# safe-autonomous-systems/fluidgym

Hardware: AMD Instinct MI355X
Metric: env-steps/sec (batched) + pressure-Poisson HBM GB/s vs roofline, 1/2/4/8 GPUs (higher is better)
Workload: dtype f32; 1 GPU; ChannelJet2D-v0 (2D channel stand-in for 'cylinder Re=100 256x128'), 64 envs/GPU, 25 PISO steps/env step, random jets, stirred by a body force N(0,2.0) redrawn every env step; global_batch=64, parallelism=env-sharded x1, 1 bcast + 1 all_gather per step (RCCL), lanes_per_gpu=2, workload_modified=True, capped_solves=0, floor_released_solves=0, advection_solver_form=two-brick, velocity_solver=on-chip Jacobi sweeps (policy advection_jacobi; 11972 solves settled by

## Files before the change

fluidgym_amd/_lib.py:

```python
from __future__ import annotations

import ctypes
import os
from ctypes import POINTER, Structure, c_char_p, c_float, c_int, c_int32, c_int64, c_void_p

_HERE = os.path.dirname(os.path.abspath(__file__))
LIB_PATH = os.environ.get("FLUIDGYM_AMD_LIB") or os.path.join(_HERE, "libfluidgym_hip.so")
LIB_F64_PATH = os.environ.get("FLUIDGYM_AMD_LIB_F64") or os.path.join(_HERE, "libfluidgym_hip_f64.so")

FG_MAX_SCALARS = 4
FG_FIELD_SUMMARY_WORK_BYTES = 128
FG_OK = 0
FG_ERR_NOT_CONVERGED = -5
FG_ERR_NOT_FINITE = -6
FG_ERR_FLUX_BALANCE = -7
FG_PERIODIC, FG_FIXED = 0, 1
FG_DIRICHLET, FG_NEUMANN = 0, 1
FG_VELOCITY, FG_PRESSURE, FG_SCALAR, FG_VELOCITY_SOURCE, FG_VISCOSITY_FIELD = 0, 1, 2, 3, 4
FG_BOUND_VELOCITY, FG_BOUND_SCALAR = 8, 16
FG_SOLVER_CG, FG_SOLVER_JACOBI, FG_SOLVER_RBGS, FG_SOLVER_MGCG, FG_SOLVER_FDCG = 0, 1, 2, 3, 4
(FG_BUF_A, FG_BUF_C_OFF, FG_BUF_ADV_RHS, FG_BUF_VEL_RESULT, FG_BUF_H, FG_BUF_DIV, FG_BUF_P_RESULT,
 FG_BUF_SCALAR_RESULT) = range(8)
FG_ERR_UNSUPPORTED = -4
FG_ERR_INVALID_ARG = -1
# ... 210 lines not shown
class FgMbSimOptions(Structure):
    _fields_ = [
        ("step", FgMbStepOptions),
        ("time_step", c_float),
        ("cfl", c_float),
        ("adaptive", c_int32),
        ("substeps", c_int32),
        ("flux_balance_tol", c_float),
        ("outflow_slot0", c_int32),
        ("outflow_count", c_int32),
        ("outflow_velm", c_float * 3),
        ("outflow_tol", c_float),
        ("max_substeps", c_int32),
        ("outflow_slot0_b", c_int32),
        ("outflow_count_b", c_int32),
    ]


(FG_MB_BUF_A, FG_MB_BUF_C_OFF, FG_MB_BUF_RHS, FG_MB_BUF_H, FG_MB_BUF_DIV, FG_MB_BUF_P_DIAG, FG_MB_BUF_P_OFF,
 FG_MB_BUF_VELOCITY_RESULT) = range(8)
FG_MB_BUF_KRYLOV0 = 8
FG_MB_BUF_PRESSURE_X = 13


class FgSimOptions(Structure):
    _fields_ = [
        ("step", FgStepOptions),
        ("time_step", c_float),
        ("cfl", c_float),
        ("adaptive", c_int32),
        ("substeps", c_int32),
        ("flux_balance_tol", c_float),
        ("outflow_mask", c_int32),
        ("outflow_velm", c_float * 3),
        ("outflow_tol", c_float),
        ("max_substeps", c_int32),
    ]


SIGNATURES = {
    "fg_abi_version": (c_int, []),
    "fg_last_error": (c_char_p, []),
    "fg_create": (c_int, [POINTER(FgConfig), POINTER(c_float), POINTER(c_float), POINTER(c_float), POINTER(c_void_p)]),
    "fg_destroy": (c_int, [c_void_p]),
    "fg_bind": (c_int, [c_void_p, c_int, c_void_p]),
    "fg_set_viscosity": (c_int, [c_void_p, c_float]),
    "fg_set_scalar_viscosity": (c_int, [c_void_p, c_int, c_float]),
    "fg_set_viscosity_batch": (c_int, [c_void_p, c_void_p]),
    "fg_set_scalar_viscosity_batch": (c_int, [c_void_p, c_int, c_void_p]),
    "fg_set_fd_preconditioner": (c_int, [c_void_p] + [POINTER(c_float)] * 7),
    "fg_max_velocity": (c_int, [c_void_p, c_void_p, c_void_p]),
    "fg_set_fd_fast_transform": (c_int, [c_void_p, c_int, c_float]),
    "fg_set_return_best": (c_int, [c_void_p, c_int]),
    "fg_set_cg_reset_steps": (c_int, [c_void_p, c_int]),
    "fg_set_advection_start": (c_int, [c_void_p, c_int]),
    "fg_set_wall_stress_forcing": (c_int, [c_void_p, c_int, c_float, c_float]),
    "fg_boundary_flux_balance": (c_int, [c_void_p, c_void_p, c_void_p]),
    "fg_step_diagnostics": (c_int, [c_void_p, POINTER(c_float), c_void_p]),
    "fg_update_advective_boundary": (c_int, [c_void_p, c_int, POINTER(c_float), c_void_p, c_void_p]),
    "fg_balance_boundary_fluxes": (c_int, [c_void_p, c_int, c_float, c_void_p, c_void_p]),
    "fg_setup_advection": (c_int, [c_void_p, c_void_p, c_int, c_int, c_void_p]),
    "fg_solve_advection": (c_int, [c_void_p, c_int, c_int, c_float, c_int, POINTER(FgSolveInfo), c_void_p]),
    "fg_copy_scalar_result_to_blocks": (c_int, [c_void_p, c_int, c_void_p]),
    "fg_setup_pressure_matrix": (c_int, [c_void_p, c_void_p]),
    "fg_setup_pressure_rhs": (c_int, [c_void_p, c_void_p, c_void_p]),
    "fg_solve_pressure": (c_int, [c_void_p, c_int, c_float, c_int, c_int, POINTER(FgSolveInfo), c_void_p]),
    "fg_correct_velocity": (c_int, [c_void_p, c_void_p]),
    "fg_copy_velocity_result_to_blocks": (c_int, [c_void_p, c_void_p]),
    "fg_copy_velocity_result_from_blocks": (c_int, [c_void_p, c_void_p]),
    "fg_piso_step": (c_int, [c_void_p, c_void_p, POINTER(FgStepOptions), POINTER(c_int32), c_void_p]),
    "fg_single_step": (c_int, [c_void_p, POINTER(FgSimOptions), POINTER(c_int32), POINTER(c_float), c_void_p]),
    "fg_multi_step": (c_int, [c_void_p, POINTER(FgSimOptions), c_int32, POINTER(c_void_p), POINTER(c_int32), POINTER(c_float), POINTER(c_int32), c_void_p]),
    "fg_make_divergence_free": (c_int, [c_void_p, c_float, c_int, POINTER(FgSolveInfo), c_void_p]),
    "fg_reset_solver_state": (c_int, [c_void_p, c_void_p]),
    "fg_solver_hints": (c_int, [c_void_p, POINTER(c_int32), c_int32]),
    "fg_env_restore_field": (c_int, [c_void_p, c_int, c_void_p, c_int32, POINTER(FgEnvSel), c_int32, c_int32, c_void_p]),
    "fg_env_reset_solver_state": (c_int, [c_void_p, POINTER(FgEnvSel), c_int32, c_void_p]),
    "fg_mb_env_restore_field": (c_int, [c_void_p, c_int, c_void_p, c_int32, POINTER(FgEnvSel), c_int32, c_int32, c_void_p]),
    "fg_mb_env_reset_solver_state": (c_int, [c_void_p, POINTER(FgEnvSel), c_int32, c_void_p]),
    "fg_mb_restore_envs": (c_int, [c_void_p, c_void_p, c_void_p, c_void_p, c_int32, POINTER(FgEnvSel), c_int32, POINTER(FgMbResetNoise),
                                   c_void_p]),
    "fg_mb_inflow_disturbance": (c_int, [c_void_p, POINTER(FgMbInflowParams), c_void_p]),
    "fg_set_pressure_refinement": (c_int, [c_void_p, c_int32, c_float, c_float]),
    "fg_get_buffer": (c_int, [c_void_p, c_int, POINTER(c_void_p), POINTER(c_int64)]),
    "fg_read_buffer": (c_int, [c_void_p, c_int, c_void_p, c_void_p]),
    "fg_poisson_apply": (c_int, [c_void_p, c_void_p, c_void_p, c_void_p, c_void_p]),
    "fg_poisson_jacobi": (c_int, [c_void_p, c_void_p, c_void_p, c_void_p, c_int, c_float, c_void_p]),
    "fg_poisson_rbgs": (c_int, [c_void_p, c_void_p, c_void_p, c_void_p, c_int, c_float, c_void_p]),
    "fg_poisson_cg": (c_int, [c_void_p, c_void_p, c_void_p, c_void_p, c_float, c_int, c_int, POINTER(FgSolveInfo),
                              c_void_p]),
    "fg_poisson_fdcg": (c_int, [c_void_p, c_void_p, c_void_p, c_void_p, c_float, c_int, c_int, POINTER(FgSolveInfo),
                                c_void_p]),
    "fg_sparse_apply_ell": (c_int, [c_void_p, c_void_p, c_int32, c_int32, c_void_p, c_int64, c_int32, c_void_p, c_void_p]),
    "fg_sparse_apply_csr": (c_int, [c_void_p, c_void_p, c_void_p, c_int32, c_void_p, c_int64, c_int32, c_void_p, c_void_p]),
    "fg_stream_triad": (c_int, [c_void_p, c_void_p, c_void_p, c_float, c_int64, c_int32, POINTER(c_float), c_void_p]),
    "fg_mb_multilevel_status": (c_int, [c_void_p, POINTER(c_int32)]),
    "fg_mb_multilevel_apply": (c_int, [c_void_p, c_void_p, c_void_p, c_void_p]),
    "fg_mb_debug_ilu_apply": (c_int, [c_void_p, c_void_p, c_void_p, c_void_p]),
    "fg_mb_debug_pressure_cg": (c_int, [c_void_p, c_float, c_int32, c_int32, POINTER(c_int32), POINTER(c_int32), POINTER(ctypes.c_double), c_void_p]),
    "fg_mb_wall_forces": (c_int, [c_void_p, c_void_p, c_void_p, c_void_p, c_int32, c_int32, c_float, c_float, c_void_p, c_void_p]),
    "fg_mb_wall_forces_batch": (c_int, [c_void_p, c_void_p, c_void_p, c_void_p, c_int32, c_int32, c_float, c_float, c_void_p, c_void_p, c_void_p]),
    "fg_mb_debug_bicgstab": (c_int, [c_void_p, c_float, c_int32, c_int32, POINTER(c_int64), POINTER(ctypes.c_double), POINTER(c_float), c_void_p]),
    "fg_dacc_host_sum": (c_int, [POINTER(ctypes.c_double), c_int64, ctypes.c_double, POINTER(ctypes.c_double)]),
    "fg_dacc_device_sum": (c_int, [POINTER(ctypes.c_double), c_int64, ctypes.c_double, c_int32, POINTER(ctypes.c_double), c_void_p]),
    "fg_field_summary": (c_int, [c_void_p, c_int32, c_int32, c_int64, c_int32, c_void_p, c_void_p, c_void_p, ctypes.c_double, ctypes.c_double,
                                 c_int32, c_void_p, c_void_p]),
# ... 238 lines not shown
```

fluidgym_amd/csrc/fg_api.hip:

```cpp
#include <stdio.h>
#include <string.h>

#include <cmath>
#include <string>
#include <vector>

#include <stdlib.h>

#include "fg_internal.h"
#include "fg_bicg.h"

static thread_local std::string g_last_error;
void fg_set_error(const std::string& msg) { g_last_error = msg; }

extern "C" int fg_abi_version(void) { return FG_ABI_VERSION; }
extern "C" const char* fg_last_error(void) { return g_last_error.c_str(); }

static FgBounds make_bounds(const fg_state* s, int channel) {
    FgBounds b;
    for (int f = 0; f < 6; ++f) {
        b.vel[f] = s->bvel[f];
        b.scal[f] = s->bscal[f];
        b.scalar_bc[f] = s->cfg.scalar_bc[f][channel < 0 ? 0 : channel];
    }
// ... 53 lines not shown
        g.h[a] = s->d_h[a]; g.rh[a] = s->d_rh[a];
    }
    const size_t BN = (size_t)g.B * g.n, d = g.dims;
    auto alloc = [&](fg_real** p, size_t count) -> hipError_t {
        hipError_t e = hipMalloc(p, sizeof(fg_real) * count);
        if (e == hipSuccess) e = hipMemset(*p, 0, sizeof(fg_real) * count);
        return e;
    };
    FG_HIP_CHECK(alloc(&s->A, BN));
    FG_HIP_CHECK(alloc(&s->rA, BN));
    FG_HIP_CHECK(alloc(&s->Coff, BN * 2 * d));
    FG_HIP_CHECK(alloc(&s->adv_rhs, BN * d));
    FG_HIP_CHECK(alloc(&s->vel_result, BN * d));
    FG_HIP_CHECK(alloc(&s->hvec, BN * d));
    FG_HIP_CHECK(alloc(&s->div, BN));
    FG_HIP_CHECK(alloc(&s->p_result, BN));
    FG_HIP_CHECK(alloc(&s->scal_result, BN));
    for (int i = 0; i < 8; ++i) FG_HIP_CHECK(alloc(&s->w[i], BN * d));
    const size_t nsys = (size_t)g.B * d;
    FG_HIP_CHECK(hipMalloc(&s->acc, sizeof(FgDacc) * nsys * FG_ACC_DOUBLES));
    FG_HIP_CHECK(hipMemset(s->acc, 0, sizeof(FgDacc) * nsys * FG_ACC_DOUBLES));
    FG_HIP_CHECK(hipMalloc(&s->flags, sizeof(int32_t) * nsys));
    FG_HIP_CHECK(hipMalloc(&s->info_dev, sizeof(fg_solve_info) * nsys));
    FG_HIP_CHECK(hipHostMalloc(&s->info_pinned, sizeof(fg_solve_info) * nsys));
    FG_HIP_CHECK(hipHostMalloc(&s->flags_pinned, sizeof(int32_t) * nsys));
    FG_HIP_CHECK(alloc(&s->scratch_B, (size_t)g.B * (4 + 2 * d)));
    FG_HIP_CHECK(hipMalloc(&s->d_bvel_ptrs, sizeof(fg_real*) * 6));
    FG_HIP_CHECK(hipMemset(s->d_bvel_ptrs, 0, sizeof(fg_real*) * 6));
    FG_HIP_CHECK(hipHostMalloc(&s->diag_pinned, sizeof(fg_real) * 2 * g.B));
    FG_HIP_CHECK(hipHostMalloc(&s->dt_pinned, sizeof(fg_real) * g.B));
    FG_HIP_CHECK(alloc(&s->dt_dev, g.B));
    FG_HIP_CHECK(hipMalloc(&s->env_sel_dev, sizeof(fg_env_sel) * g.B));
    s->t_rem_dev = nullptr;
#if !FG_F64
    FG_HIP_CHECK(hipMalloc(&s->t_rem_dev, sizeof(double) * g.B));
    FG_HIP_CHECK(hipMemset(s->t_rem_dev, 0, sizeof(double) * g.B));
#endif
    if (int rc = fg_poll_create(&s->poll, (int)(nsys > 2 * (size_t)g.B ? nsys : 2 * (size_t)g.B))) return rc;
    for (int k = 0; k < 4; ++k) { s->pred_bicg[k] = 2; s->pred_cg[k] = 1; }
    s->wall_forcing_axis = -1;
    s->ref64_inner = 1e-4f;
    s->fd_row_epoch = -1; s->rA_epoch = 0; s->fd_row_part_epoch = -1;
    for (int k = 0; k < 4; ++k) s->jac_hist[k] = FgJacHist{0, 0, 0};
    s->jac_solves = s->jac_fallbacks = 0;
    FG_HIP_CHECK(hipHostMalloc(&s->jac_prev, sizeof(float) * 4 * nsys));
    s->jac_rA_epoch = -1;
    FG_HIP_CHECK(hipMalloc(&s->fcg_alpha, sizeof(double) * 2 * (size_t)g.B));
    FG_HIP_CHECK(hipMemset(s->fcg_alpha, 0, sizeof(double) * 2 * (size_t)g.B));
    FG_HIP_CHECK(hipMalloc(&s->fcg_xsum, sizeof(FgDacc) * 2 * (size_t)g.B));
    FG_HIP_CHECK(hipMemset(s->fcg_xsum, 0, sizeof(FgDacc) * 2 * (size_t)g.B));
    FG_HIP_CHECK(hipMalloc(&s->fcg_lazy, sizeof(int32_t) * (size_t)g.B));
    FG_HIP_CHECK(hipMemset(s->fcg_lazy, 0, sizeof(int32_t) * (size_t)g.B));
    s->cg_return_best = 1;
    s->cg_reset_steps = 100;
    s->adv_from_result = 1;
    FG_HIP_CHECK(hipMalloc(&s->cg_acc, sizeof(FgDacc) * (size_t)g.B * 8 * 64));
    FG_HIP_CHECK(hipMemset(s->cg_acc, 0, sizeof(FgDacc) * (size_t)g.B * 8 * 64));
    FG_HIP_CHECK(hipMalloc(&s->cg_best.best_crit, sizeof(fg_real) * g.B));
    FG_HIP_CHECK(hipMalloc(&s->cg_best.saved_crit, sizeof(fg_real) * g.B));
    FG_HIP_CHECK(hipMalloc(&s->cg_best.save_at, sizeof(int32_t) * g.B));
    FG_HIP_CHECK(alloc(&s->cg_best.best_x, BN));
    *out = s;
    return FG_OK;
}

extern "C" int fg_destroy(fg_handle s) {
    if (!s) return FG_OK;
    for (int a = 0; a < 3; ++a) { (void)hipFree(s->d_h[a]); (void)hipFree(s->d_rh[a]); }
    fg_real* owned[] = {s->A, s->rA, s->Coff, s->adv_rhs, s->vel_result, s->hvec, s->div, s->p_result, s->scal_result,
                      s->scratch_B};
    for (fg_real* p : owned) (void)hipFree(p);
    for (int i = 0; i < 8; ++i) (void)hipFree(s->w[i]);
    (void)hipFree(s->acc); (void)hipFree(s->flags); (void)hipFree(s->info_dev);
    (void)hipHostFree(s->info_pinned); (void)hipHostFree(s->flags_pinned);
    fg_prof_destroy(s);
    fg_poll_destroy(&s->poll);
    (void)hipFree(s->d_bvel_ptrs); (void)hipHostFree(s->diag_pinned); (void)hipHostFree(s->dt_pinned); (void)hipFree(s->dt_dev); (void)hipFree(s->t_rem_dev); (void)hipFree(s->env_sel_dev);
    float* fd[] = {s->fd_Qx, s->fd_QxT, s->fd_Qz, s->fd_QzT, s->fd_lower, s->fd_inv, s->fd_cp};
    for (float* p : fd) if (p) (void)hipFree(p);
    if (s->fd_dct_tw) { (void)hipFree(s->fd_dct_tw); (void)hipFree(s->fd_dct_rot); }
    (void)hipFree(s->cg_acc); (void)hipFree(s->fcg_alpha); (void)hipFree(s->fcg_xsum); (void)hipFree(s->fcg_lazy);
    if (s->jac_prev) (void)hipHostFree(s->jac_prev);
    (void)hipFree(s->fd_row_part); (void)hipFree(s->fd_lam_x); (void)hipFree(s->fd_row_inv); (void)hipFree(s->fd_row_cp); (void)hipFree(s->fd_row_lower);
    (void)hipFree(s->line_inv); (void)hipFree(s->line_cp); (void)hipFree(s->ilu_d);
    (void)hipFree(s->r64_buf); (void)hipFree(s->r64_acc); (void)hipFree(s->ref64_x); (void)hipFree(s->force_uniform);
    (void)hipFree(s->fd_lam); (void)hipFree(s->helm_diag); (void)hipFree(s->helm_lower); (void)hipFree(s->helm_upper); (void)hipFree(s->helm_tmp); (void)hipFree(s->helm_lower_row); (void)hipFree(s->helm_lower_row2); (void)hipFree(s->line_inv2); (void)hipFree(s->line_cp2);
    (void)hipFree(s->cg_best.best_crit); (void)hipFree(s->cg_best.saved_crit); (void)hipFree(s->cg_best.save_at); (void)hipFree(s->cg_best.best_x);
    delete s;
    return FG_OK;
}

static int sync_bvel_ptrs(fg_state* s);
extern "C" int fg_bind(fg_handle s, int field, fg_real* ptr) {
    FG_REQUIRE(s, FG_ERR_INVALID_ARG, "null handle");
    if (field == FG_VELOCITY) s->velocity = ptr;
    else if (field == FG_PRESSURE) s->pressure = ptr;
    else if (field == FG_SCALAR) s->scalar = ptr;
    else if (field == FG_VELOCITY_SOURCE) s->velocity_source = ptr;
    else if (field == FG_VISCOSITY_FIELD) s->visc_field = ptr;
    else if (field >= FG_BOUND_VELOCITY && field < FG_BOUND_VELOCITY + 6) {
        s->bvel[field - FG_BOUND_VELOCITY] = ptr;
        return sync_bvel_ptrs(s);
    }
    else if (field >= FG_BOUND_SCALAR && field < FG_BOUND_SCALAR + 6) s->bscal[field - FG_BOUND_SCALAR] = ptr;
    else FG_REQUIRE(false, FG_ERR_INVALID_ARG, "fg_bind: unknown field id");
    return FG_OK;
}

extern "C" int fg_set_viscosity(fg_handle s, fg_real v) {
    FG_REQUIRE(s, FG_ERR_INVALID_ARG, "null handle");
    s->viscosity = v;
    return FG_OK;
}
extern "C" int fg_set_scalar_viscosity(fg_handle s, int ch, fg_real v) {
    FG_REQUIRE(s && ch >= 0 && ch < FG_MAX_SCALARS, FG_ERR_INVALID_ARG, "bad channel");
    s->scalar_viscosity[ch] = v;
    s->scalar_viscosity_set = true;
    return FG_OK;
}
extern "C" int fg_set_viscosity_batch(fg_handle s, const fg_real* nu_B) {
    FG_REQUIRE(s, FG_ERR_INVALID_ARG, "null handle");
    s->viscosity_B = nu_B;
    s->helm_pre_mask = 0;
    return FG_OK;
}
extern "C" int fg_set_scalar_viscosity_batch(fg_handle s, int ch, const fg_real* k_B) {
    FG_REQUIRE(s && ch >= 0 && ch < FG_MAX_SCALARS, FG_ERR_INVALID_ARG, "bad channel");
    s->scalar_viscosity_B[ch] = k_B;
    s->helm_pre_mask = 0;
    return FG_OK;
}

extern "C" int fg_set_fd_preconditioner(fg_handle s, const float* Qx, const float* QxT, const float* Qz, const float* QzT,
                                        const float* lower, const float* inv, const float* cp) {
    FG_REQUIRE(s && Qx && QxT && lower && inv && cp, FG_ERR_INVALID_ARG, "null argument");
    FG_REQUIRE(s->grid.fixed[2] && s->grid.fixed[3], FG_ERR_UNSUPPORTED, "FD preconditioner needs FIXED y faces");
    FG_REQUIRE(s->grid.dims == 2 || (Qz && QzT), FG_ERR_INVALID_ARG, "Qz required in 3-D");
#if !FG_F64
    FG_REQUIRE(s->grid.ny <= 640, FG_ERR_UNSUPPORTED, "FD preconditioner: at most 640 cells along y (LDS of the tridiagonal solve)");
#endif
    const size_t nx = s->grid.nx, ny = s->grid.ny, nz = s->grid.nz;
    auto up = [&](float** dst, const float* src, size_t count) -> hipError_t {
        if (*dst) (void)hipFree(*dst);
        hipError_t e = hipMalloc(dst, sizeof(float) * count);
        if (e == hipSuccess) e = hipMemcpy(*dst, src, sizeof(float) * count, hipMemcpyHostToDevice);
        return e;
    };
    FG_HIP_CHECK(up(&s->fd_Qx, Qx, nx * nx));
    FG_HIP_CHECK(up(&s->fd_QxT, QxT, nx * nx));
    if (s->grid.dims == 3) {
        FG_HIP_CHECK(up(&s->fd_Qz, Qz, nz * nz));
        FG_HIP_CHECK(up(&s->fd_QzT, QzT, nz * nz));
    }
    FG_HIP_CHECK(up(&s->fd_lower, lower, ny));
    FG_HIP_CHECK(up(&s->fd_inv, inv, nx * ny * nz));
    FG_HIP_CHECK(up(&s->fd_cp, cp, nx * ny * nz));
    s->fd_dct_x = 0;
    return FG_OK;
}

extern "C" int fg_set_return_best(fg_handle s, int on) {
    FG_REQUIRE(s, FG_ERR_INVALID_ARG, "null handle");
    s->cg_return_best = on ? 1 : 0;
    return FG_OK;
}

extern "C" int fg_set_cg_reset_steps(fg_handle s, int steps) {
    FG_REQUIRE(s && steps >= 0, FG_ERR_INVALID_ARG, "fg_set_cg_reset_steps: null handle or negative step count");
    s->cg_reset_steps = steps;
    return FG_OK;
}

extern "C" int fg_set_advection_start(fg_handle s, int from_result) {
    FG_REQUIRE(s, FG_ERR_INVALID_ARG, "null handle");
    s->adv_from_result = from_result ? 1 : 0;
    return FG_OK;
}

extern "C" int fg_set_wall_stress_forcing(fg_handle s, int axis, fg_real coef_lo, fg_real coef_hi) {
    FG_REQUIRE(s, FG_ERR_INVALID_ARG, "null handle");
    FG_REQUIRE(axis < s->grid.dims, FG_ERR_INVALID_ARG, "fg_set_wall_stress_forcing: bad axis");
    if (axis >= 0) {
        FG_REQUIRE(s->grid.fixed[2] && s->grid.fixed[3], FG_ERR_UNSUPPORTED, "fg_set_wall_stress_forcing: needs FIXED y faces (walls)");
        if (!s->force_uniform) {
            FG_HIP_CHECK(hipMalloc(&s->force_uniform, sizeof(fg_real) * (size_t)s->grid.B * s->grid.dims));
            FG_HIP_CHECK(hipMemset(s->force_uniform, 0, sizeof(fg_real) * (size_t)s->grid.B * s->grid.dims));
        }
    }
    s->wall_forcing_axis = axis; s->wall_forcing_coef[0] = coef_lo; s->wall_forcing_coef[1] = coef_hi;
    return FG_OK;
}

extern "C" int fg_set_advection_preconditioner(fg_handle s, int mode) {
    FG_REQUIRE(s, FG_ERR_INVALID_ARG, "null handle");
    FG_REQUIRE(mode >= 0 && mode <= 5, FG_ERR_INVALID_ARG, "fg_set_advection_preconditioner: mode must be 0 (off), 1 (line, always), 2 (line, fallback), 3 (Helmholtz, always), 4 (ILU(0), always) or 5 (ILU(0), fallback)");
    FG_REQUIRE(mode != 3 || s->fd_lam != nullptr, FG_ERR_INVALID_ARG, "fg_set_advection_preconditioner: mode 3 needs fg_set_fd_helmholtz");
    if (mode >= 4) { if (int rc = fg_ilu_alloc(s)) return rc; }
    else if (mode != 0)
        if (int rc = fg_line_alloc(s)) return rc;
    s->adv_precond = mode;
    return FG_OK;
}
extern "C" int fg_set_advection_jacobi(fg_handle s, int on) {
    FG_REQUIRE(s, FG_ERR_INVALID_ARG, "null handle");
    if (!s->adv_jacobi_env) s->adv_jacobi = on ? 1 : 0;
    for (int k = 0; k < 4; ++k) s->jac_hist[k] = FgJacHist{0, 0, 0};
    return FG_OK;
}
extern "C" int fg_advection_jacobi_counts(fg_handle s, int64_t* out2) {
    FG_REQUIRE(s && out2, FG_ERR_INVALID_ARG, "null argument");
    out2[0] = s->jac_solves; out2[1] = s->jac_fallbacks;
    return FG_OK;
}
extern "C" int fg_set_double_fallback(fg_handle s, int on) {
    FG_REQUIRE(s, FG_ERR_INVALID_ARG, "null handle");
    s->double_fallback = on ? 1 : 0;
// ... 191 lines not shown
            s->fd_row_part_epoch = s->rA_epoch;
        }
#endif
        if (buoy_axis >= 0) {
            a.buoy_T = s->scalar; a.buoy_stride = (long)s->cfg.n_scalars * s->grid.n; a.buoy_axis = buoy_axis; a.buoy_factor = buoy_factor;
            a.source_w = s->velocity_source;
        }
    }
    return fg_launch_adv_build(s, make_bounds(s, channel), a, (hipStream_t)stream);
}

static int advection_solve(fg_state* s, FgBicgArgs a, fg_solve_info* info, hipStream_t st, int for_scalar = 0, int channel = 0, bool* spec_ran = nullptr);

extern "C" int fg_solve_advection(fg_handle s, int for_scalar, int channel, fg_real tol, int max_iterations,
                                  fg_solve_info* info_host, void* stream) {
    FG_REQUIRE(s, FG_ERR_INVALID_ARG, "null handle");
    FgBicgArgs a;
    a.diag = s->A; a.off = s->Coff; a.rhs = s->adv_rhs;
    a.dt = s->cur_dt;
    a.tol = tol; a.max_iterations = max_iterations;
    if (for_scalar) { a.x = s->scal_result; a.nc = 1; a.use_x0 = 0; a.kind = 0; }
    else { a.x = s->vel_result; a.nc = s->grid.dims; a.use_x0 = s->adv_from_result; }
    return advection_solve(s, a, info_host, (hipStream_t)stream, for_scalar, channel);
}

extern "C" int fg_copy_scalar_result_to_blocks(fg_handle s, int channel, void* stream) {
    FG_REQUIRE(s && s->scalar, FG_ERR_NOT_BOUND, "scalar not bound");
    const int n = s->grid.n;
    if (s->cfg.n_scalars == 1) return fg_launch_copy_active(s, s->cur_dt, s->scal_result, s->scalar, 1, (hipStream_t)stream);
    FG_HIP_CHECK(hipMemcpy2DAsync(s->scalar + (size_t)channel * n, sizeof(fg_real) * n * s->cfg.n_scalars, s->scal_result,
                                  sizeof(fg_real) * n, sizeof(fg_real) * n, s->grid.B, hipMemcpyDeviceToDevice,
                                  (hipStream_t)stream));
    return FG_OK;
}

extern "C" int fg_setup_pressure_matrix(fg_handle s, void* stream) {
    FG_REQUIRE(s, FG_ERR_INVALID_ARG, "null handle");
    s->rA_epoch++;
    return fg_launch_pressure_setup(s, s->cur_dt, (hipStream_t)stream);
}

extern "C" int fg_setup_pressure_rhs(fg_handle s, const fg_real* dt_B, void* stream) {
    FG_REQUIRE(s && dt_B, FG_ERR_INVALID_ARG, "null argument");
    if (int rc = check_bound(s, false)) return rc;
    hipStream_t st = (hipStream_t)stream;
    if (int rc = fg_launch_h(s, dt_B, s->vel_result, st)) return rc;
    return fg_launch_div(s, make_bounds(s, 0), dt_B, s->hvec, s->div, st);
}

struct SpecH { fg_state* s; const fg_real* dt; const fg_step_options* opt; hipStream_t st; };
static int spec_h(void* p) {
    const SpecH* c = static_cast<const SpecH*>(p);
    fg_state* s = c->s;
    if (int rc = fg_launch_h(s, c->dt, s->vel_result, c->st)) return rc;
    return fg_launch_div(s, make_bounds(s, 0), c->dt, s->hvec, s->div, c->st, !c->opt->pressure_warm_start,
                         c->opt->pressure_method == FG_SOLVER_FDCG && s->fd_Qx != nullptr);
}

static int launch_corrector(fg_state* s, const fg_real* dt, const FgCgOutcome& o, bool last, hipStream_t st) {
    const bool mean_folded = last && o.mean_ready;
    FG_REQUIRE(!o.lazy_z || !last || mean_folded, FG_ERR_UNSUPPORTED, "fg_piso_step: an unmaterialised pressure without its folded mean");
    if (last && !mean_folded)
        if (int rc = fg_launch_mean_sub(s, dt, s->p_result, s->pressure, st)) return rc;
    const FgMeanRef mean = {s->fcg_xsum, s->info_dev, s->pressure, o.marks_valid ? s->fcg_lazy : nullptr, s->fcg_alpha};
    const FgLazyRef lazy = {s->fcg_lazy, s->fcg_alpha, last ? s->p_result : nullptr};
    const fg_real* p = o.lazy_z ? o.lazy_z : ((last && !mean_folded) ? s->pressure : s->p_result);
    return fg_launch_correct(s, dt, s->rA, s->hvec, p, s->vel_result, st, last ? s->velocity : nullptr, mean_folded ? &mean : nullptr, o.lazy_z ? &lazy : nullptr);
}

struct SpecCorrect { fg_state* s; const fg_real* dt; bool last; hipStream_t st; };
static int spec_correct(void* p, const FgCgOutcome& o) {
    const SpecCorrect* c = static_cast<const SpecCorrect*>(p);
    return launch_corrector(c->s, c->dt, o, c->last, c->st);
}

static int solve_pressure(fg_state* s, const fg_real* dt, int method, fg_real tol, int max_iterations, int use_previous,
                          fg_solve_info* info_host, hipStream_t st, bool finalize = true, int kind = 2, FgCgOutcome* out = nullptr,
                          FgCgSpec spec = FgCgSpec{}) {
    int rc = FG_OK;
    FgCgOutcome own;
    if (!out) out = &own;
    if (method == FG_SOLVER_CG || method == FG_SOLVER_FDCG) {
        FgCgArgs a;
        a.rA = s->rA; a.b = s->div; a.x = s->p_result;
        a.r = s->w[0]; a.p = s->w[1]; a.Ap = s->w[2];
        a.dt = dt; a.tol = tol; a.max_iterations = max_iterations; a.use_x0 = use_previous;
        a.reset_steps = s->cg_reset_steps;
        a.precond = (method == FG_SOLVER_FDCG);
        a.kind = kind;
        a.check_every = a.precond ? 2 : 16;
        a.lazy_ok = finalize ? 0 : 1;
        a.spec = spec;
#if !FG_F64
        if (s->ref64_outer > 0) a.lazy_ok = 0;
#endif
        rc = fg_cg_solve(s, a, info_host, st, out);
#if !FG_F64
        if (s->ref64_outer > 0 && (rc == FG_OK || rc == FG_ERR_NOT_CONVERGED)) rc = fg_refine64_pressure(s, a, info_host, st, out);
        if (s->double_fallback && (rc == FG_ERR_NOT_FINITE || (s->ladder_force & 2))) {
            std::vector<fg_solve_info> tmp;
            fg_solve_info* info = info_host;
            if (!info) { tmp.assign(s->info_pinned, s->info_pinned + s->grid.B); info = tmp.data(); }
            s->rung_count[2] += 1;
            rc = fg_rung64_cg(s, a, info, (s->ladder_force & 2) != 0, st, out);
        }
#endif
    } else {
        fg_set_error("fg_solve_pressure: only FG_SOLVER_CG drives the PISO step (Jacobi/RBGS are smoothers)");
        return FG_ERR_UNSUPPORTED;
// ... 89 lines not shown
    int status = FG_OK;
    auto soft = [&](int rc) {
        if (rc == FG_ERR_NOT_CONVERGED) { status = rc; return FG_OK; }
        return rc;
    };
#if !FG_F64
    const bool sweeps_first = s->adv_linesweep && s->grid.dims == 2 && s->jac_hist[0].skip == 0 && s->jac_hist[1].skip == 0;
    if (scalar && s->cfg.n_scalars == 1 && s->adv_precond == 3 && s->fd_lam && !s->visc_field && !sweeps_first) {
        const FgNu nu2[2] = {fg_nu(s, 1, 0), fg_nu(s)};
        const int wlo[2] = {s->cfg.scalar_bc[2][0] == FG_DIRICHLET, 1}, whi[2] = {s->cfg.scalar_bc[3][0] == FG_DIRICHLET, 1};
        if (int rc = fg_helm_factor_pair(s, dt_B, nu2, wlo, whi, st)) return rc;
    }
#endif
    if (scalar) {
        FgRange range_scalar("scalar_advection");
        for (int ch = 0; ch < s->cfg.n_scalars; ++ch) {
            if (int rc = fg_setup_advection(s, dt_B, 1, ch, stream)) return rc;
            FgBicgArgs a;
            a.diag = s->A; a.off = s->Coff; a.rhs = s->adv_rhs; a.x = s->scal_result; a.nc = 1;
            a.dt = dt_B; a.tol = opt->advection_tol; a.max_iterations = opt->max_iterations; a.use_x0 = 0; a.kind = 0;
            if (int rc = soft(advection_solve(s, a, info.data(), st, 1, ch))) return rc;
            const int m = max_iters(info.data(), B);
            stats[0] = m > stats[0] ? m : stats[0];
            s->ctr.add(0, info.data(), B);
            const int n = s->grid.n;
            if (s->cfg.n_scalars == 1) {
                if (int rc = fg_launch_copy_active(s, dt_B, s->scal_result, s->scalar, 1, st)) return rc;
            } else {
                (void)n;
                fg_set_error("multi-channel scalar copy with inactive envs not implemented");
                return FG_ERR_UNSUPPORTED;
            }
        }
    }
    fg_range_push("velocity_assembly_and_solve");
    struct PopOnce { bool armed = true; void fire() { if (armed) { fg_range_pop(); armed = false; } } ~PopOnce() { fire(); } } range_velocity;
    if (int rc = setup_advection(s, dt_B, 0, 0, stream, opt->buoyancy_axis, opt->buoyancy_factor)) return rc;
    bool h_div_ran = false;
    {
        FgBicgArgs a;
        a.diag = s->A; a.off = s->Coff; a.rhs = s->adv_rhs; a.x = s->vel_result; a.nc = d;
        a.dt = dt_B; a.tol = opt->advection_tol; a.max_iterations = opt->max_iterations; a.use_x0 = s->adv_from_result;
        SpecH spec_h_ctx = {s, dt_B, opt, st};
        if (opt->corrector_steps > 0) a.spec = FgSpecHook{spec_h, &spec_h_ctx};
        if (int rc = soft(advection_solve(s, a, info.data(), st, 0, 0, &h_div_ran))) return rc;
        stats[1] = max_iters(info.data(), B * d);
        s->ctr.add(1, info.data(), B * d);
    }
    range_velocity.fire();
    for (int c = 0; c < opt->corrector_steps; ++c) {
        FgRange range_corr(c == 0 ? "pressure_corrector_0" : "pressure_corrector_1+");
        const bool last = (c + 1 == opt->corrector_steps);
        if (!(c == 0 && h_div_ran)) {
            if (int rc = fg_launch_h(s, dt_B, s->vel_result, st)) return rc;
            if (int rc = fg_launch_div(s, make_bounds(s, 0), dt_B, s->hvec, s->div, st, !opt->pressure_warm_start,
                                       opt->pressure_method == FG_SOLVER_FDCG && s->fd_Qx != nullptr))
                return rc;
        }
        SpecCorrect spec_ctx = {s, dt_B, last, st};
        FgCgOutcome outcome;
        if (int rc = soft(solve_pressure(s, dt_B, opt->pressure_method, opt->pressure_tol, opt->max_iterations, opt->pressure_warm_start ? 1 : 0,
                                         info.data(), st, false, c == 0 ? 0 : 1, &outcome, FgCgSpec{spec_correct, &spec_ctx})))
            return rc;
        if (c < 2) { stats[2 + c] = max_iters(info.data(), B); s->ctr.add(2 + c, info.data(), B); }
        if (!outcome.spec_done)
            if (int rc = launch_corrector(s, dt_B, outcome, last, st)) return rc;
    }
    if (opt->corrector_steps <= 0)
        if (int rc = fg_launch_copy_active(s, dt_B, s->vel_result, s->velocity, d, st)) return rc;
    if (stats_host) memcpy(stats_host, stats, sizeof(stats));
    s->ctr.piso_steps += 1;
    return status;
}

extern "C" int fg_config_dump(fg_handle s, char* buf, int n) {
    FG_REQUIRE(s && buf && n > 0, FG_ERR_INVALID_ARG, "fg_config_dump: bad argument");
    std::string out = std::string("{\"build\": \"") + (FG_F64 ? "f64" : "f32") + "\"";
    fg_switches_json(s, out);
    const std::pair<const char*, long long> state[] = {
        {"fast_transform_x", s->fd_dct_x}, {"fd_preconditioner", s->fd_Qx ? 1 : 0}, {"helmholtz", s->fd_lam ? 1 : 0}, {"advection_preconditioner", s->adv_precond},
        {"advection_from_result", s->adv_from_result}, {"return_best", s->cg_return_best}, {"cg_reset_steps", s->cg_reset_steps}, {"double_fallback", s->double_fallback},
        {"wall_forcing_axis", s->wall_forcing_axis}, {"first_iterate_polls", s->fcg_first_polls}, {"unstored_pressure_solves", s->fcg_unstored},
        {"jacobi_speculation_misses", s->jac_spec_missed}, {"jacobi_floor_released", s->jac_floor_released}, {"pressure_refinement_corrections", s->ref64_corrections}};
    for (const auto& kv : state) fg_json_put(out, kv.first, kv.second);
    return fg_json_out(out + "}", buf, n);
}

extern "C" int fg_solver_unconverged(fg_handle s, int64_t* out4) {
    FG_REQUIRE(s != nullptr && out4 != nullptr, FG_ERR_INVALID_ARG, "fg_solver_unconverged: bad argument");
    for (int k = 0; k < 4; ++k) out4[k] = s->ctr.unconv[k];
    return FG_OK;
}

extern "C" int fg_solver_counters(fg_handle s, int64_t* out13, int32_t reset) {
    FG_REQUIRE(s != nullptr, FG_ERR_INVALID_ARG, "fg_solver_counters: null handle");
    if (out13) s->ctr.write(out13);
    if (reset) s->ctr.reset();
    return FG_OK;
}

extern "C" int fg_single_step(fg_handle s, const fg_sim_options* o, int32_t* out, fg_real* flux_host, void* stream);
extern "C" int fg_multi_step(fg_handle s, const fg_sim_options* o, int32_t n, const fg_real* const* bvel_schedule, int32_t* out_6n,
                             fg_real* flux_host, int32_t* steps_done, void* stream) {
    FG_REQUIRE(s && o && out_6n && n >= 0, FG_ERR_INVALID_ARG, "fg_multi_step: bad argument");
    if (steps_done) *steps_done = 0;
    for (int k = 0; k < n; ++k) {
        if (bvel_schedule)
            for (int f = 0; f < 2 * s->grid.dims; ++f)
                if (const fg_real* p = bvel_schedule[(size_t)k * 6 + f])
                    if (int rc = fg_bind(s, FG_BOUND_VELOCITY + f, const_cast<fg_real*>(p))) return rc;
        if (int rc = fg_single_step(s, o, out_6n + 6 * (size_t)k, flux_host, stream)) return rc;
        if (steps_done) *steps_done = k + 1;
        if (out_6n[6 * (size_t)k + 5] == 0 && !s->cg_return_best) break;
    }
    return FG_OK;
}

static inline bool is_close_zero(double a) { return std::fabs(a) <= 1e-8; }

extern "C" int fg_single_step(fg_handle s, const fg_sim_options* o, int32_t* out, fg_real* flux_host, void* stream) {
    fg_htrace("single_step_in");
    FgRange range_sim("fg_single_step");
    FG_REQUIRE(s && o && out, FG_ERR_INVALID_ARG, "null argument");
    if (int rc = check_bound(s, o->step.advect_scalar && s->cfg.n_scalars > 0)) return rc;
    hipStream_t st = (hipStream_t)stream;
    const int B = s->grid.B;
    const FgBounds bnd = make_bounds(s, 0);
    std::vector<double> t_rem(B, (double)o->time_step);
    int32_t stats[4] = {-1, -1, -1, -1};
    int substeps = 0, all_ok = 1;
    bool first = true;
    int fixed_left = o->adaptive ? 0 : (o->substeps > 0 ? o->substeps : 1);
    for (;;) {
        bool any = false;
        if (o->adaptive) {
            for (int b = 0; b < B; ++b) any = any || (t_rem[b] > 0 && !is_close_zero(t_rem[b]));
// ... 71 lines not shown
            fg_real velm3[3] = {o->outflow_velm[0], o->outflow_velm[1], o->outflow_velm[2]};
            if (int rc = fg_launch_balance(s, bnd, o->outflow_mask, (fg_real)0.01 * o->outflow_tol, s->dt_dev, st, folded ? o->outflow_mask : 0, velm3,
                                           dt_by_value ? s->dt_pinned : nullptr))
                return rc;
        }
        int rc = fg_piso_step(s, s->dt_dev, &o->step, stats, stream);
        if (rc == FG_ERR_NOT_CONVERGED) all_ok = 0;
        else if (rc != FG_OK) return rc;
        if (deferred) {
            if (int rc2 = fg_poll_wait_words(&s->poll, po_cfl, 12 * B, first ? 2 * B : B, st)) return rc2;
            for (int b = 0; b < B; ++b) {
                s->diag_pinned[B + b] = fg_poll_word_float(&s->poll, 12 * B + b);
                if (first) s->diag_pinned[b] = fg_poll_word_float(&s->poll, 13 * B + b);
            }
            if (first) if (int rc2 = flux_guard()) return rc2;
            for (int b = 0; b < B; ++b) s->dt_pinned[b] = advance(b, s->diag_pinned[B + b]);
        }
        ++substeps;
        first = false;
        if (!o->adaptive) --fixed_left;
        if (substeps >= (o->max_substeps > 0 ? o->max_substeps : 100000)) break;
    }
    fg_htrace("single_step_out");
    for (int i = 0; i < 4; ++i) out[i] = stats[i];
    out[4] = substeps;
    out[5] = all_ok;
    return FG_OK;
}

extern "C" int fg_make_divergence_free(fg_handle s, fg_real tol, int max_iterations, fg_solve_info* info_host,
                                       void* stream) {
    FG_REQUIRE(s, FG_ERR_INVALID_ARG, "null handle");
    if (int rc = check_bound(s, false)) return rc;
    s->cur_dt = nullptr;
    hipStream_t st = (hipStream_t)stream;
    const size_t BN = (size_t)s->grid.B * s->grid.n;
    std::vector<fg_real> ones(BN, 1.f);
    FG_HIP_CHECK(hipMemcpyAsync(s->rA, ones.data(), sizeof(fg_real) * BN, hipMemcpyHostToDevice, st));
    s->rA_epoch++;
    FG_HIP_CHECK(hipStreamSynchronize(st));
    if (int rc = fg_launch_copy_active(s, nullptr, s->velocity, s->hvec, s->grid.dims, st)) return rc;
    if (int rc = fg_launch_div(s, make_bounds(s, 0), nullptr, s->hvec, s->div, st)) return rc;
    int rc = solve_pressure(s, nullptr, FG_SOLVER_CG, tol, max_iterations, 0, info_host, st);
    if (rc != FG_OK && rc != FG_ERR_NOT_CONVERGED) return rc;
    if (int rc2 = fg_launch_correct(s, nullptr, s->rA, s->hvec, s->pressure, s->vel_result, st)) return rc2;
    if (int rc2 = fg_launch_copy_active(s, nullptr, s->vel_result, s->velocity, s->grid.dims, st)) return rc2;
    return rc;
}

extern "C" int fg_reset_solver_state(fg_handle s, void* stream) {
    FG_REQUIRE(s && s->velocity, FG_ERR_NOT_BOUND, "velocity not bound");
    for (int k = 0; k < 4; ++k) s->jac_hist[k] = FgJacHist{0, 0, 0};
    FG_HIP_CHECK(hipMemsetAsync(s->p_result, 0, sizeof(fg_real) * (size_t)s->grid.B * s->grid.n, (hipStream_t)stream));
    return fg_launch_copy_active(s, nullptr, s->velocity, s->vel_result, s->grid.dims, (hipStream_t)stream);
}

extern "C" int fg_solver_hints(fg_handle s, int32_t* hints12, int32_t set) {
    FG_REQUIRE(s != nullptr && hints12 != nullptr, FG_ERR_INVALID_ARG, "fg_solver_hints: bad argument");
    for (int k = 0; k < 4; ++k) {
        FgJacHist& H = s->jac_hist[k];
        if (set) { H.sweeps = hints12[3 * k]; H.skip = hints12[3 * k + 1]; H.fails = hints12[3 * k + 2]; }
        else { hints12[3 * k] = H.sweeps; hints12[3 * k + 1] = H.skip; hints12[3 * k + 2] = H.fails; }
    }
    return FG_OK;
}

extern "C" int fg_get_buffer(fg_handle s, int which, fg_real** out_ptr, int64_t* out_count) {
    FG_REQUIRE(s && out_ptr && out_count, FG_ERR_INVALID_ARG, "null argument");
    const int64_t BN = (int64_t)s->grid.B * s->grid.n, d = s->grid.dims;
    switch (which) {
        case FG_BUF_A: *out_ptr = s->A; *out_count = BN; break;
        case FG_BUF_C_OFF: *out_ptr = s->Coff; *out_count = BN * 2 * d; break;
        case FG_BUF_ADV_RHS: *out_ptr = s->adv_rhs; *out_count = BN * d; break;
        case FG_BUF_VEL_RESULT: *out_ptr = s->vel_result; *out_count = BN * d; break;
        case FG_BUF_H: *out_ptr = s->hvec; *out_count = BN * d; break;
        case FG_BUF_DIV: *out_ptr = s->div; *out_count = BN; break;
        case FG_BUF_P_RESULT: *out_ptr = s->p_result; *out_count = BN; break;
        case FG_BUF_SCALAR_RESULT: *out_ptr = s->scal_result; *out_count = BN; break;
        default:
            if (which >= 100 && which < 108) { *out_ptr = s->w[which - 100]; *out_count = BN * d; break; }
            FG_REQUIRE(false, FG_ERR_INVALID_ARG, "unknown buffer id");
    }
    return FG_OK;
}

extern "C" int fg_read_buffer(fg_handle s, int which, fg_real* dst, void* stream) {
    fg_real* src = nullptr;
    int64_t count = 0;
    if (int rc = fg_get_buffer(s, which, &src, &count)) return rc;
    FG_REQUIRE(dst, FG_ERR_INVALID_ARG, "null destination");
    FG_HIP_CHECK(hipMemcpyAsync(dst, src, sizeof(fg_real) * count, hipMemcpyDeviceToDevice, (hipStream_t)stream));
    return FG_OK;
}

extern "C" int fg_poisson_apply(fg_handle s, const fg_real* rA, const fg_real* x, fg_real* y, void* stream) {
    FG_REQUIRE(s && rA && x && y, FG_ERR_INVALID_ARG, "null argument");
    return fg_poisson_apply_launch(s, rA, x, y, (hipStream_t)stream);
}

extern "C" int fg_poisson_jacobi(fg_handle s, const fg_real* rA, const fg_real* b, fg_real* x, int n_sweeps, fg_real omega,
                                 void* stream) {
    FG_REQUIRE(s && rA && b && x && n_sweeps >= 0, FG_ERR_INVALID_ARG, "bad argument");
    hipStream_t st = (hipStream_t)stream;
    fg_real* buf[2] = {x, s->w[5]};
    for (int i = 0; i < n_sweeps; ++i)
        if (int rc = fg_poisson_jacobi_launch(s, rA, b, buf[i & 1], buf[(i + 1) & 1], omega, st)) return rc;
// ... 53 lines not shown
```

fluidgym_amd/csrc/fg_cg.h:

```cpp
#pragma once
#include "fg_internal.h"

#define FG_CG_SLOTS 64
#define FG_CG_NAMES 8

#ifdef __HIPCC__
__device__ __forceinline__ FgDacc* fg_acc_ptr(FgDacc* acc, int b, int name) {
    return acc + ((size_t)b * FG_CG_NAMES + name) * FG_CG_SLOTS;
}
__device__ __forceinline__ double fg_acc_total(const FgDacc* a, int ns) {
    if (ns == 1) return acc_ld(a + (0));
    const int lane = threadIdx.x & 63;
    double v = (lane < ns) ? acc_ld(a + (lane)) : 0.0;
#pragma unroll
    for (int o = 32; o > 0; o >>= 1) v += __shfl_xor(v, o, 64);
    return v;
}
__device__ __forceinline__ void fg_acc_zero(FgDacc* a, int ns) {
    const int lane = threadIdx.x & 63;
    if (lane < ns) acc_st(a + (lane), 0.0);
}
__device__ __forceinline__ void fg_acc_add(FgDacc* a, int ns, unsigned tile, double v) {
    acc_add(a + (tile & (unsigned)(ns - 1)), v);
}
#endif

struct FgCgBegin { FgDacc* acc; int32_t* flags; fg_solve_info* info; FgDacc* mean_sums; FgBest best; int track_best, ns;
                   FgDacc* xsum; };
int fg_cg_slots(const fg_state* s);
#ifdef __HIPCC__
__device__ __forceinline__ void fg_cg_begin_env(const FgCgBegin& q, const fg_real* __restrict__ dt, int b) {
    for (int k = threadIdx.x; k < FG_CG_NAMES * q.ns; k += blockDim.x)
        acc_st(fg_acc_ptr(q.acc, b, k / q.ns) + k % q.ns, 0.0);
    if (threadIdx.x != 0) return;
    acc_st(q.mean_sums + b, 0.0);
    if (q.xsum) { acc_st(q.xsum + 2 * b, 0.0); acc_st(q.xsum + 2 * b + 1, 0.0); }
    q.best.best_crit[b] = q.track_best ? INFINITY : 0.f;
    q.best.saved_crit[b] = INFINITY;
    q.best.save_at[b] = -1;
    const bool active = (dt == nullptr) || (dt[b] > 0.f);
    flag_st(q.flags + (b), active ? 0 : 3);
    q.info[b].final_residual = 0.f;
    q.info[b].used_iterations = -1;
    q.info[b].converged = active ? 0 : 1;
    q.info[b].is_finite = 1;
}
#endif

struct FgCgStart { FgDacc* acc; fg_real* r; fg_real* x; int ns; };

struct FgCgJudge {
    FgDacc* acc;
    int32_t* flags; fg_solve_info* info;
    fg_real tol; int it, n, ns;
};
#ifdef __HIPCC__
__device__ __forceinline__ bool fg_cg_judge(const FgCgJudge& j, int b, bool leader) {
    const double rr = fg_acc_total(fg_acc_ptr(j.acc, b, (j.it + 1) % 3), j.ns);
    const fg_real crit = (fg_real)sqrt(rr / (double)j.n);
    if (crit >= j.tol) return false;
    if (leader) {
        const bool finite = isfinite(crit);
        j.info[b].final_residual = crit;
        j.info[b].used_iterations = j.it;
        j.info[b].converged = finite ? 1 : 0;
        j.info[b].is_finite = finite ? 1 : 0;
        flag_st(j.flags + (b), finite ? 1 : 2);
    }
    return true;
}
#endif

struct FgCgLead { FgCgJudge judge; FgBest best; };
#ifdef __HIPCC__
__device__ __forceinline__ bool fg_cg_lead(const FgCgLead& q, int b, bool lead_block) {
    const FgCgJudge& j = q.judge;
    const double rr = fg_acc_total(fg_acc_ptr(j.acc, b, (j.it + 1) % 3), j.ns);
    const fg_real crit = (fg_real)sqrt(rr / (double)j.n);
    const bool done = !(crit >= j.tol);
    if (lead_block && threadIdx.x < 64) {
        if (!done) fg_acc_zero(fg_acc_ptr(j.acc, b, (j.it + 2) % 3), j.ns);
        if (threadIdx.x == 0) {
            j.info[b].final_residual = crit;
            j.info[b].used_iterations = j.it;
            if (done) {
                const bool finite = isfinite(crit);
                j.info[b].converged = finite ? 1 : 0;
                j.info[b].is_finite = finite ? 1 : 0;
                flag_st(j.flags + (b), finite ? 1 : 2);
            } else {
                fg_best_decide(q.best, b, crit, j.it + 1);
            }
        }
    }
    return done;
}
#endif
```

fluidgym_amd/csrc/fg_fftcg.h:

```cpp
#pragma once
#include "fg_internal.h"
#include "fg_cg.h"

constexpr int FCG_DELTA = 3, FCG_GAMMA = 5;

struct FcgVectors {
    fg_real* z; fg_real* w;
    fg_real* p; fg_real* s;
    fg_real* x; fg_real* r; fg_real* t1;
};

struct FcgUpdArgs {
    const float* z; const float* w; float* p; float* s; float* x; float* r; float* t1;
    const float2* tw; const float2* rot; float fs0, fs;
    const int32_t* flags; FgDacc* acc; double* alpha; FgDacc* xsum; FgBest best;
    int ns, rows, it, first; long env_stride;
    const float* r0; int x_zero;
    const int32_t* lazy;
};
struct FcgInvArgs {
    const float* u; const float* r; const float* rA; float* z; float* w;
    const float2* tw; const float2* rot; float is0, is;
    const int32_t* flags; FgDacc* acc; int ns, rows, it; long env_stride;
    const float* hy; const float* rhy; const float* hx; const float* rhx; int fixed_x;
    FgDacc* xsum; int extras;
};

struct FcgDivArgs {
    const float* h; float* div; float* r; float* x; float* t1;
    const float* bvel[4];
    const float2* tw; const float2* rot; float fs0, fs;
    const float* dt; FgDacc* acc; int ns, rows; long n;
    const float* hx; const float* hy; int fixed_x;
};

#if !FG_F64
int fg_fcg_div_fwd(fg_state* s, const FgBounds& bnd, const fg_real* dt, const fg_real* hvec, fg_real* div, int ns, hipStream_t st);
bool fg_fcg_ok(const fg_state* s);
int fg_fcg_update_fwd(fg_state* s, const FcgVectors& v, int it, int first, int ns, hipStream_t st, bool marks_valid, const fg_real* r0 = nullptr);
int fg_fcg_inv_apply(fg_state* s, const FcgVectors& v, const fg_real* rA, int it, int ns, hipStream_t st, int extras = 0);
int fg_fcg_check0(fg_state* s, fg_real tol, int ns, hipStream_t st, FgPollOut poll, bool* marks_valid);
#endif
```

fluidgym_amd/csrc/fg_fftcg.hip:

```cpp
#include "fg_internal.h"
#include "fg_cg.h"
#include "fg_fftrow.h"
#include "fg_fftcg.h"

#if !FG_F64
namespace {

using fgfft::Map;

template <int N, bool PERIODIC>
__global__ __launch_bounds__(256) void k_fcg_update_fwd(FcgUpdArgs a) {
    constexpr int EPL = N / 64;
    __shared__ __attribute__((aligned(16))) float2 buf[2][4][N];
    __shared__ __attribute__((aligned(16))) float2 twl[N];
    __shared__ float red[8];
    const int b = blockIdx.y;
    const int lane = threadIdx.x & 63, wave = threadIdx.x >> 6;
    if (a.flags[b] != 0) {
        if (a.lazy && a.lazy[b] == 1) {
            const float alpha = (float)a.alpha[b * 2];
            const int row0 = 2 * (blockIdx.x * 4 + wave);
#pragma unroll
            for (int half = 0; half < 2; ++half) {
                const int row = row0 + half;
// ... 307 lines not shown
        const int jc = live ? j : 0;
        const float hy = a.hy[jc];
        const bool at_lo = jc == 0, at_hi = jc == a.rows - 1;
        const float* sr = sx + half * N;
        float* out = half ? db : da;
#pragma unroll
        for (int q = 0; q < M::NG; ++q) {
            const int i0 = q * 64 * VW + lane * VW;
            float hc[VW], v1[VW], vu[VW], vd[VW], hx[VW], bl[VW], bh[VW];
            fgfft::ldv<VW>(sr + i0, hc);
            fgfft::ldv<VW>(a.h + hb1 + (size_t)jc * N + i0, v1);
            fgfft::ldv<VW>(a.h + hb1 + (size_t)(at_lo ? jc : jc - 1) * N + i0, vu);
            fgfft::ldv<VW>(a.h + hb1 + (size_t)(at_hi ? jc : jc + 1) * N + i0, vd);
            fgfft::ldv<VW>(a.hx + i0, hx);
            if (at_lo) fgfft::ldv<VW>(a.bvel[2] + ((size_t)b * 2 + 1) * N + i0, bl);
            if (at_hi) fgfft::ldv<VW>(a.bvel[3] + ((size_t)b * 2 + 1) * N + i0, bh);
            const float hl = sr[(i0 == 0) ? N - 1 : i0 - 1], hr = sr[(i0 + VW == N) ? 0 : i0 + VW];
            const bool xlo = (i0 == 0) && a.fixed_x, xhi = (i0 + VW == N) && a.fixed_x;
#pragma unroll
            for (int e = 0; e < VW; ++e) {
                const float h_l = (e == 0) ? hl : hc[e > 0 ? e - 1 : 0], h_r = (e == VW - 1) ? hr : hc[e < VW - 1 ? e + 1 : VW - 1];
                float acc = 0.f;
                {
                    const float area = hy;
                    const float F_hi = (e == VW - 1 && xhi) ? a.bvel[1][((size_t)b * 2 + 0) * a.rows + jc] * area : 0.5f * (hc[e] + h_r) * area;
                    const float F_lo = (e == 0 && xlo) ? a.bvel[0][((size_t)b * 2 + 0) * a.rows + jc] * area : 0.5f * (hc[e] + h_l) * area;
                    acc += F_hi - F_lo;
                }
                {
                    const float area = hx[e];
                    const float F_hi = at_hi ? bh[e] * area : 0.5f * (v1[e] + vd[e]) * area;
                    const float F_lo = at_lo ? bl[e] * area : 0.5f * (v1[e] + vu[e]) * area;
                    acc += F_hi - F_lo;
                }
                out[q * VW + e] = live ? acc : 0.f;
            }
        }
        if (live) {
#pragma unroll
            for (int e = 0; e < EPL; ++e) part[0] += out[e] * out[e];
            const size_t o = (size_t)b * a.n + (size_t)j * N;
            fgfft::store_row<N>(a.div + o, lane, half ? db : da);
        }
    }
    __syncthreads();
    float oa[EPL], ob[EPL];
    fgfft::forward_rows<N, PERIODIC>(da, db, oa, ob, buf[0][wave], buf[1][wave], twl, a.rot, fgfft::Scales{a.fs0, a.fs}, lane);
    if (row0 < a.rows) fgfft::store_row<N>(a.t1 + (size_t)b * a.n + (size_t)row0 * N, lane, oa);
    if (row0 + 1 < a.rows) fgfft::store_row<N>(a.t1 + (size_t)b * a.n + (size_t)(row0 + 1) * N, lane, ob);
    fg_block_sum<1>(part, red);
    if (threadIdx.x == 0) fg_acc_add(fg_acc_ptr(a.acc, b, 0), a.ns, blockIdx.x, (double)part[0]);
}

template <bool PERIODIC>
int launch_upd(const fg_state* s, int slot, int n, const FcgUpdArgs& a, dim3 grid, hipStream_t st) {
    switch (n) {
        case 64: FG_LAUNCH_P(s, slot, (k_fcg_update_fwd<64, PERIODIC>), grid, dim3(256), 0, st, a); break;
        case 128: FG_LAUNCH_P(s, slot, (k_fcg_update_fwd<128, PERIODIC>), grid, dim3(256), 0, st, a); break;
        case 256: FG_LAUNCH_P(s, slot, (k_fcg_update_fwd<256, PERIODIC>), grid, dim3(256), 0, st, a); break;
        case 512: FG_LAUNCH_P(s, slot, (k_fcg_update_fwd<512, PERIODIC>), grid, dim3(256), 0, st, a); break;
        default: fg_set_error("fused CG: unsupported row length"); return FG_ERR_UNSUPPORTED;
    }
    return FG_OK;
}
template <bool PERIODIC>
int launch_inv(const fg_state* s, int slot, int n, const FcgInvArgs& a, dim3 grid, hipStream_t st) {
    switch (n) {
        case 64: FG_LAUNCH_P(s, slot, (k_fcg_inv_apply<64, PERIODIC>), grid, dim3(320), 0, st, a); break;
        case 128: FG_LAUNCH_P(s, slot, (k_fcg_inv_apply<128, PERIODIC>), grid, dim3(320), 0, st, a); break;
        case 256: FG_LAUNCH_P(s, slot, (k_fcg_inv_apply<256, PERIODIC>), grid, dim3(320), 0, st, a); break;
        case 512: FG_LAUNCH_P(s, slot, (k_fcg_inv_apply<512, PERIODIC>), grid, dim3(320), 0, st, a); break;
        default: fg_set_error("fused CG: unsupported row length"); return FG_ERR_UNSUPPORTED;
    }
    return FG_OK;
}

template <bool PERIODIC>
int launch_div(const fg_state* s, int n, const FcgDivArgs& a, dim3 grid, hipStream_t st) {
    const int slot = fg_prof_slot(s, FG_PK_DIV, nullptr, s->grid.B, 28.0 * (double)s->grid.n, (8.0 + 5.0 * log2((double)n)) * (double)s->grid.n, st);
    switch (n) {
        case 64: FG_LAUNCH_P(s, slot, (k_fcg_div_fwd<64, PERIODIC>), grid, dim3(256), 0, st, a); break;
        case 128: FG_LAUNCH_P(s, slot, (k_fcg_div_fwd<128, PERIODIC>), grid, dim3(256), 0, st, a); break;
        case 256: FG_LAUNCH_P(s, slot, (k_fcg_div_fwd<256, PERIODIC>), grid, dim3(256), 0, st, a); break;
        case 512: FG_LAUNCH_P(s, slot, (k_fcg_div_fwd<512, PERIODIC>), grid, dim3(256), 0, st, a); break;
        default: fg_set_error("fused CG: unsupported row length"); return FG_ERR_UNSUPPORTED;
    }
    return FG_OK;
}

}

bool fg_fcg_ok(const fg_state* s) {
    const FgGrid& G = s->grid;
    return s->cg_fused && s->fd_dct_x != 0 && G.dims == 2 && fg_fd_dct_supported(G.nx) && G.fixed[2] && G.fixed[3] && G.ny >= 3 &&
           s->fcg_alpha != nullptr;
}

int fg_fcg_update_fwd(fg_state* s, const FcgVectors& v, int it, int first, int ns, hipStream_t st, bool marks_valid, const fg_real* r0) {
    const FgGrid& G = s->grid;
    FcgUpdArgs a = {};
    a.r0 = r0; a.x_zero = r0 ? 1 : 0;
    a.lazy = (it == 0 && marks_valid) ? s->fcg_lazy : nullptr;
    a.z = v.z; a.w = v.w; a.p = v.p; a.s = v.s; a.x = v.x; a.r = v.r; a.t1 = v.t1;
    a.tw = s->fd_dct_tw; a.rot = s->fd_dct_rot; a.fs0 = s->fd_dct_fwd[0]; a.fs = s->fd_dct_fwd[1];
    a.flags = s->flags; a.acc = s->cg_acc; a.alpha = s->fcg_alpha; a.xsum = s->fcg_xsum; a.best = s->cg_best;
    a.ns = ns; a.rows = G.ny; a.it = it; a.first = first; a.env_stride = G.n;
    const dim3 grid((G.ny + 7) / 8, G.B);
    const int slot = fg_prof_slot(s, FG_PK_FCG_UPD, s->flags, G.B, (first ? (r0 ? 24.0 : 28.0) : 44.0) * G.n, (10.0 + 5.0 * log2((double)G.nx)) * G.n, st);
    if (int rc = (s->fd_dct_x == 2 ? launch_upd<true>(s, slot, G.nx, a, grid, st) : launch_upd<false>(s, slot, G.nx, a, grid, st))) return rc;
    FG_HIP_CHECK(hipGetLastError());
    return FG_OK;
}

int fg_fcg_inv_apply(fg_state* s, const FcgVectors& v, const fg_real* rA, int it, int ns, hipStream_t st, int extras) {
    const FgGrid& G = s->grid;
    FcgInvArgs a = {};
    a.u = v.t1; a.r = v.r; a.rA = rA; a.z = v.z; a.w = v.w;
    a.tw = s->fd_dct_tw; a.rot = s->fd_dct_rot; a.is0 = s->fd_dct_inv[0]; a.is = s->fd_dct_inv[1];
    a.flags = s->flags; a.acc = s->cg_acc; a.ns = ns; a.rows = G.ny; a.it = it; a.env_stride = G.n;
    a.xsum = s->fcg_xsum; a.extras = (extras && it == 0) ? 1 : 0;
    a.hy = G.h[1]; a.rhy = G.rh[1]; a.hx = G.h[0]; a.rhx = G.rh[0]; a.fixed_x = G.fixed[0];
    const dim3 grid((G.ny + 7) / 8, G.B);
    const int slot = fg_prof_slot(s, FG_PK_FCG_INV, s->flags, G.B, 20.0 * G.n, (14.0 + 5.0 * log2((double)G.nx)) * G.n, st);
    if (int rc = (s->fd_dct_x == 2 ? launch_inv<true>(s, slot, G.nx, a, grid, st) : launch_inv<false>(s, slot, G.nx, a, grid, st))) return rc;
    FG_HIP_CHECK(hipGetLastError());
    return FG_OK;
}
int fg_fcg_check0(fg_state* s, fg_real tol, int ns, hipStream_t st, FgPollOut poll, bool* marks_valid) {
    const FgGrid& G = s->grid;
    hipLaunchKernelGGL(k_fcg_check0, dim3((G.B + CHECK_WAVES - 1) / CHECK_WAVES), dim3(64 * CHECK_WAVES), 0, st, s->cg_acc, s->flags, s->info_dev, s->info_pinned, s->fcg_alpha, s->fcg_lazy,
                       tol, G.n, G.B, ns, poll);
    FG_HIP_CHECK(hipGetLastError());
    *marks_valid = true;
    return FG_OK;
}
int fg_fcg_div_fwd(fg_state* s, const FgBounds& bnd, const fg_real* dt, const fg_real* hvec, fg_real* div, int ns, hipStream_t st) {
    const FgGrid& G = s->grid;
    FcgDivArgs a = {};
    a.h = hvec; a.div = div; a.r = s->w[0]; a.x = s->p_result; a.t1 = s->w[3];
    for (int f = 0; f < 4; ++f) a.bvel[f] = bnd.vel[f];
    a.tw = s->fd_dct_tw; a.rot = s->fd_dct_rot; a.fs0 = s->fd_dct_fwd[0]; a.fs = s->fd_dct_fwd[1];
    a.dt = dt; a.acc = s->cg_acc; a.ns = ns; a.rows = G.ny; a.n = G.n;
    a.hx = G.h[0]; a.hy = G.h[1]; a.fixed_x = G.fixed[0];
    const dim3 grid((G.ny + 7) / 8, G.B);
    if (int rc = (s->fd_dct_x == 2 ? launch_div<true>(s, G.nx, a, grid, st) : launch_div<false>(s, G.nx, a, grid, st))) return rc;
    FG_HIP_CHECK(hipGetLastError());
    return FG_OK;
}
#endif
```

fluidgym_amd/csrc/fg_internal.h:

```cpp
#pragma once
#include <hip/hip_runtime.h>
#include <hip/hip_ext.h>
#include <math.h>
#include <stdint.h>
#include <cstring>
#include <string>
#include <type_traits>

#include "../../include/fluidgym_hip.h"
#include "fg_switches.h"

#ifdef FG_REAL_DOUBLE
struct alignas(16) fg_real4 { double x, y, z, w; };
__host__ __device__ __forceinline__ fg_real4 make_fg_real4(double x, double y, double z, double w) { fg_real4 r; r.x = x; r.y = y; r.z = z; r.w = w; return r; }
#define FG_F64 1
#define FG_FMAX fmax
#define FG_FABS fabs
#define FG_SQRT sqrt
#else
typedef float4 fg_real4;
#define make_fg_real4 make_float4
#define FG_F64 0
#define FG_FMAX fmaxf
#define FG_FABS fabsf
// ... 250 lines not shown
    return c;
}

template <int DIMS, int VEC>
struct FgNbr {
    FgVec<VEC> c, xm, xp, ym, yp, zm, zp;
};

#if !FG_F64
__device__ __forceinline__ float fg_dpp_from_lane_before(float v) {
    return __int_as_float(__builtin_amdgcn_update_dpp(0, __float_as_int(v), 0x111, 0xf, 0xf, true));
}
__device__ __forceinline__ float fg_dpp_from_lane_after(float v) {
    return __int_as_float(__builtin_amdgcn_update_dpp(0, __float_as_int(v), 0x101, 0xf, 0xf, true));
}
#endif
template <int DIMS, int VEC>
__device__ __forceinline__ void fg_x_neighbours(const fg_real* __restrict__ q, const FgCtx<DIMS, VEC>& c, const FgVec<VEC>& ctr,
                                                fg_real& left, fg_real& right) {
#if !FG_F64
    if constexpr (VEC == 4) {
        const int lx = threadIdx.x & 15;
        left = fg_dpp_from_lane_before(ctr.v[3]);
        right = fg_dpp_from_lane_after(ctr.v[0]);
        if (lx == 0 || c.ixm != c.idx - 1) left = q[c.ixm];
        if (lx == 15 || c.ixp != c.idx + VEC) right = q[c.ixp];
        return;
    }
#endif
    left = q[c.ixm];
    right = q[c.ixp];
}

template <int DIMS, int VEC>
__device__ __forceinline__ FgNbr<DIMS, VEC> fg_gather(const fg_real* __restrict__ q, const FgCtx<DIMS, VEC>& c) {
    FgNbr<DIMS, VEC> n;
    n.c = fg_load<VEC>(q + c.idx);
    fg_real left, right;
    fg_x_neighbours<DIMS, VEC>(q, c, n.c, left, right);
#pragma unroll
    for (int e = 0; e < VEC; ++e) {
        n.xm.v[e] = (e == 0) ? left : n.c.v[e - 1];
        n.xp.v[e] = (e == VEC - 1) ? right : n.c.v[e + 1];
    }
    n.ym = fg_load<VEC>(q + c.iym);
    n.yp = fg_load<VEC>(q + c.iyp);
    if constexpr (DIMS == 3) {
        n.zm = fg_load<VEC>(q + c.izm);
        n.zp = fg_load<VEC>(q + c.izp);
    }
    return n;
}

template <int DIMS, int VEC>
__device__ __forceinline__ void fg_gather_axis(const fg_real* __restrict__ q, const FgCtx<DIMS, VEC>& c, int axis,
                                               FgVec<VEC>& ctr, FgVec<VEC>& lo, FgVec<VEC>& hi) {
    ctr = fg_load<VEC>(q + c.idx);
    if (axis == 0) {
        fg_real left, right;
        fg_x_neighbours<DIMS, VEC>(q, c, ctr, left, right);
#pragma unroll
        for (int e = 0; e < VEC; ++e) {
            lo.v[e] = (e == 0) ? left : ctr.v[e - 1];
            hi.v[e] = (e == VEC - 1) ? right : ctr.v[e + 1];
        }
    } else if (axis == 1) {
        lo = fg_load<VEC>(q + c.iym);
        hi = fg_load<VEC>(q + c.iyp);
    } else {
        lo = fg_load<VEC>(q + c.izm);
        hi = fg_load<VEC>(q + c.izp);
    }
}

template <int DIMS, int VEC>
struct FgMetric {
    fg_real hx[VEC], rhx[VEC];
    fg_real rhx_m, rhx_p;
    fg_real hy, rhy, rhy_m, rhy_p;
    fg_real hz, rhz, rhz_m, rhz_p;
};

template <int DIMS, int VEC>
__device__ __forceinline__ FgMetric<DIMS, VEC> fg_metrics(const FgGrid& g, const FgCtx<DIMS, VEC>& c) {
    FgMetric<DIMS, VEC> m;
#pragma unroll
    for (int e = 0; e < VEC; ++e) {
        m.hx[e] = g.h[0][c.i0 + e];
        m.rhx[e] = g.rh[0][c.i0 + e];
    }
    m.rhx_m = g.rh[0][(c.i0 == 0) ? g.nx - 1 : c.i0 - 1];
    m.rhx_p = g.rh[0][(c.i0 + VEC == g.nx) ? 0 : c.i0 + VEC];
    m.hy = g.h[1][c.j];
    m.rhy = g.rh[1][c.j];
    m.rhy_m = g.rh[1][(c.j == 0) ? g.ny - 1 : c.j - 1];
    m.rhy_p = g.rh[1][(c.j == g.ny - 1) ? 0 : c.j + 1];
    if constexpr (DIMS == 3) {
        m.hz = g.h[2][c.k];
        m.rhz = g.rh[2][c.k];
        m.rhz_m = g.rh[2][(c.k == 0) ? g.nz - 1 : c.k - 1];
        m.rhz_p = g.rh[2][(c.k == g.nz - 1) ? 0 : c.k + 1];
    } else {
        m.hz = m.rhz = m.rhz_m = m.rhz_p = 1.f;
    }
    return m;
}
// ... 150 lines not shown
int fg_solve_infos_report(const fg_state* s, int count, fg_solve_info* info_host, int* used_max);
inline uint32_t fg_poll_word(const FgPoll* P, int i) { return (uint32_t)(__atomic_load_n(P->gran + i, __ATOMIC_RELAXED) & 0xffffffffull); }
inline float fg_poll_word_float(const FgPoll* P, int i) { const uint32_t u = fg_poll_word(P, i); float f; memcpy(&f, &u, 4); return f; }
inline void fg_poll_info(const FgPoll* P, int sys, fg_solve_info* out) {
    const uint32_t w = fg_poll_word(P, 2 * sys + 1);
    out->final_residual = fg_poll_word_float(P, 2 * sys);
    out->used_iterations = (int32_t)(w >> 2) - 1; out->converged = (w >> 1) & 1; out->is_finite = w & 1;
}
void fg_htrace(const char* tag);
void fg_range_push(const char* name);
void fg_range_pop();
struct FgRange { explicit FgRange(const char* name) { fg_range_push(name); } ~FgRange() { fg_range_pop(); } FgRange(const FgRange&) = delete; FgRange& operator=(const FgRange&) = delete; };

struct FgBest {
    fg_real* best_crit;
    fg_real* saved_crit;
    int32_t* save_at;
    fg_real* best_x;
};
#ifdef __HIPCC__
__device__ __forceinline__ void fg_best_decide(const FgBest& best, int b, fg_real crit, int it) {
    if (it >= 1 && crit < 0.5f * best.best_crit[b]) {
        best.best_crit[b] = crit;
        best.saved_crit[b] = crit;
        best.save_at[b] = it;
    }
}
#endif

struct FgCounters {
    long long sum[4] = {0, 0, 0, 0}, n[4] = {0, 0, 0, 0}, piso_steps = 0;
    long long unconv[4] = {0, 0, 0, 0};
    int max[4] = {0, 0, 0, 0};
    void add(int kind, const fg_solve_info* info, int count) {
        for (int i = 0; i < count; ++i) {
            const int it = info[i].used_iterations;
            if (it < 0 && info[i].final_residual == 0.f) continue;
            const int v = it + 1;
            sum[kind] += v; n[kind] += 1; max[kind] = v > max[kind] ? v : max[kind];
            if (!info[i].converged) unconv[kind] += 1;
        }
    }
    void reset() { *this = FgCounters(); }
    void write(int64_t* out) const {
        for (int k = 0; k < 4; ++k) { out[k] = sum[k]; out[4 + k] = n[k]; out[8 + k] = max[k]; }
        out[12] = piso_steps;
    }
};

struct FgPrepared {
    int bicg_nc; const fg_real* bicg_dt;
    int cg_ns, cg_best; const fg_real* cg_dt;
    int cg_start;
    void clear() { *this = FgPrepared{}; }
    void set_bicg(int nc, const fg_real* dt) { clear(); bicg_nc = nc; bicg_dt = dt; }
    void set_cg(int ns, int best, const fg_real* dt) { clear(); cg_ns = ns; cg_best = best; cg_dt = dt; }
    bool cg_for(const fg_real* dt) const { return cg_ns > 0 && cg_dt == dt; }
    void set_cg_start(int form) { cg_start = form; }
    bool take_bicg(int nc, const fg_real* dt) { const bool ready = bicg_nc == nc && bicg_dt == dt; clear(); return ready; }
    int take_cg(int ns, int best, const fg_real* dt) {
        const int got = (cg_ns == ns && cg_best == best && cg_dt == dt) ? cg_start : -1; clear(); return got;
    }
};

struct FgNu {
    fg_real v = 0; const fg_real* per_env = nullptr;
#ifdef __HIPCC__
    __device__ __forceinline__ fg_real at(int b) const { return per_env ? per_env[b] : v; }
#endif
    bool same(const FgNu& o) const { return v == o.v && per_env == o.per_env; }
};

struct fg_state {
    fg_config cfg;
    FgGrid grid;
    int vec;
    fg_real viscosity;
    fg_real scalar_viscosity[FG_MAX_SCALARS];
    bool scalar_viscosity_set;
    const fg_real* viscosity_B;
    const fg_real* scalar_viscosity_B[FG_MAX_SCALARS];
    fg_real* d_h[3];
    fg_real* d_rh[3];
    fg_real* velocity;
    fg_real* pressure;
    fg_real* scalar;
    fg_real* velocity_source;
    fg_real* visc_field;
    fg_real* bvel[6];
    fg_real* bscal[6];
    fg_real* A;
    fg_real* rA;
    fg_real* Coff;
    fg_real* adv_rhs;
    fg_real* vel_result;
    fg_real* hvec;
    fg_real* div;
    fg_real* p_result;
    fg_real* scal_result;
    fg_real* w[8];
    FgDacc* acc;
    int32_t* flags;
    fg_solve_info* info_dev;
    fg_solve_info* info_pinned;
    int32_t* flags_pinned;
    fg_real* scratch_B;
    FgProf prof;
    FgDacc* cg_acc;
    FgBest cg_best;
    int cg_return_best;
    int cg_reset_steps;
    int adv_from_result;
    int adv_precond; long long line_retries;
    int wall_forcing_axis; fg_real wall_forcing_coef[2]; fg_real* force_uniform;
    FG_SB_SWITCHES(FG_SW_MEMBER)
    double* fcg_alpha; FgDacc* fcg_xsum;
    int32_t* fcg_lazy;
    long jac_spec_missed;
    long jac_floor_released = 0;
    long fcg_unstored, fcg_first_polls;
    fg_real* line_inv; fg_real* line_cp;
    fg_real* ilu_d;
    int double_fallback; int ladder_force; long long rung_count[4];
    double* r64_buf; FgDacc* r64_acc;
    int ref64_outer; float ref64_tol, ref64_inner; double* ref64_x; long ref64_corrections;
    float* fd_Qx; float* fd_QxT; float* fd_Qz; float* fd_QzT; float* fd_lower; float* fd_inv; float* fd_cp;
    float* fd_lam; float* helm_diag; float* helm_lower; float* helm_upper; float* helm_tmp;
    float* helm_lower_row; float helm_rs; int helm_cb;
    float* line_inv2; float* line_cp2; float* helm_lower_row2; int helm_pre_mask; const fg_real* helm_pre_dt; FgNu helm_pre_nu[2]; int helm_pre_walls[2][2]; int helm_set;
    int fd_dct_x; float2* fd_dct_tw; float2* fd_dct_rot; float fd_dct_fwd[2]; float fd_dct_inv[2];
    float* fd_lam_x; float* fd_row_inv; float* fd_row_cp; float* fd_row_lower; long fd_row_epoch; mutable long rA_epoch;
    float* fd_row_part; long fd_row_part_epoch;
    int32_t* forms_rec;
    const fg_real* adv_last_dt;
    fg_real** d_bvel_ptrs;
    fg_real* diag_pinned;
    fg_real* dt_pinned;
    fg_real* dt_dev;
    double* t_rem_dev;
    int pred_bicg[4], pred_cg[4];
    int adv_jacobi, adv_jacobi_env; FgJacHist jac_hist[4]; float* jac_prev;
    long long jac_solves, jac_fallbacks;
    long jac_rA_epoch;
    FgCounters ctr;
    const fg_real* cur_dt;
    FgPoll poll;
    mutable int maxvel_clean;
    FgPrepared prepared;
    fg_env_sel* env_sel_dev;
    size_t n_cells() const { return (size_t)grid.n; }
};
inline FgNu fg_nu(const fg_state* s, int for_scalar = 0, int channel = 0) {
    FgNu n;
    if (for_scalar && s->scalar_viscosity_B[channel]) { n.v = s->scalar_viscosity[channel]; n.per_env = s->scalar_viscosity_B[channel]; }
    else if (for_scalar && s->scalar_viscosity_set) n.v = s->scalar_viscosity[channel];
    else { n.v = s->viscosity; n.per_env = s->viscosity_B; }
    return n;
}

void fg_set_error(const std::string& msg);
#define FG_REQUIRE(cond, code, msg)  \
    do {                             \
        if (!(cond)) {               \
            fg_set_error(msg);       \
            return code;             \
        }                            \
    } while (0)
#define FG_HIP_CHECK(expr)                                                                        \
    do {                                                                                          \
        hipError_t _e = (expr);                                                                   \
// ... 10 lines not shown
        else { constexpr int DIMS = 3, VEC = 1; __VA_ARGS__; }                    \
    } while (0)
#else
#define FG_DISPATCH(s, ...)                                                       \
    do {                                                                          \
        if ((s)->grid.dims == 2) {                                                \
            if ((s)->vec == 4) { constexpr int DIMS = 2, VEC = 4; __VA_ARGS__; }  \
            else { constexpr int DIMS = 2, VEC = 1; __VA_ARGS__; }                \
        } else {                                                                  \
            if ((s)->vec == 4) { constexpr int DIMS = 3, VEC = 4; __VA_ARGS__; }  \
            else { constexpr int DIMS = 3, VEC = 1; __VA_ARGS__; }                \
        }                                                                         \
    } while (0)
#endif

struct FgBicgBegin { FgDacc* acc; fg_real* sc; int32_t* flags; fg_solve_info* info; int nc; };
#ifdef __HIPCC__
__device__ __forceinline__ void fg_bicg_begin_sys(const FgBicgBegin& q, const fg_real* __restrict__ dt, int sys) {
    for (int k = 0; k < FG_ACC_DOUBLES; ++k) acc_st(q.acc + ((size_t)sys * FG_ACC_DOUBLES + k), 0.0);
    sc_st(q.sc + (sys * 2), 1.f); sc_st(q.sc + (sys * 2 + 1), 1.f);
    const bool active = (dt == nullptr) || (dt[sys / q.nc] > 0.f);
    flag_st(q.flags + (sys), active ? 0 : 3);
    q.info[sys].final_residual = 0.f;
    q.info[sys].used_iterations = -1;
    q.info[sys].converged = active ? 0 : 1;
    q.info[sys].is_finite = 1;
}
#endif
struct FgAdvArgs {
    const fg_real* vel;
    const fg_real* scal;
    long scal_env_stride;
    const fg_real* source;
    const fg_real* force;
    const fg_real* dt;
    FgNu nu;
    const fg_real* visc;
    int for_scalar;
    int channel, n_scalars;
    fg_real* A; fg_real* Coff; fg_real* rhs;
    fg_real* rA;
    FgBicgBegin begin;
    const fg_real* buoy_T; long buoy_stride; int buoy_axis; fg_real buoy_factor; fg_real* source_w;
    fg_real* row_part;
};
int fg_launch_adv_build(fg_state* s, const FgBounds& bnd, const FgAdvArgs& a, hipStream_t st);
int fg_launch_wall_forcing(const fg_state* s, hipStream_t st);
int fg_launch_sgs(const fg_state* s, const FgBounds& bnd, fg_real coefficient, fg_real* out, hipStream_t st);
int fg_launch_pressure_setup(const fg_state* s, const fg_real* dt, hipStream_t st);
int fg_launch_h(fg_state* s, const fg_real* dt, const fg_real* vel_result, hipStream_t st);
int fg_launch_div(fg_state* s, const FgBounds& bnd, const fg_real* dt, const fg_real* hvec, fg_real* div, hipStream_t st,
                  bool cg_from_zero = false,
                  bool fused_fwd = false);
struct FgMeanRef { const FgDacc* sums; const fg_solve_info* info; fg_real* p_copy; const int32_t* lazy; const double* alpha; };
struct FgLazyRef { const int32_t* lazy; const double* alpha; fg_real* p_res; };
int fg_launch_correct(const fg_state* s, const fg_real* dt, const fg_real* rA, const fg_real* hvec, const fg_real* p,
                      fg_real* vel_out, hipStream_t st, fg_real* vel_copy = nullptr, const FgMeanRef* mean = nullptr, const FgLazyRef* lazy = nullptr);
struct FgDtRule { double* t_rem; fg_real* dt_out; float cfl; double time_step; int reset; };
int fg_launch_max_velocity(const fg_state* s, const FgBounds& bnd, fg_real* out_B, hipStream_t st, fg_real* mirror_B = nullptr,
                           FgPollOut poll = FgPollOut{nullptr, 0}, fg_real* flux_B = nullptr, fg_real* flux_mirror = nullptr,
                           FgDtRule rule = FgDtRule{nullptr, nullptr, 0.f, 0.0, 0});
int fg_launch_flux_balance(const fg_state* s, const FgBounds& bnd, fg_real* out_B, hipStream_t st, FgPollOut poll = FgPollOut{nullptr, 0});
int fg_launch_copy_active(const fg_state* s, const fg_real* dt, const fg_real* src, fg_real* dst, int comps, hipStream_t st);
int fg_launch_buoyancy(const fg_state* s, const fg_real* dt, const fg_real* T, long t_env_stride, fg_real* source, int axis,
                       fg_real factor, hipStream_t st);
int fg_launch_outflow(const fg_state* s, int face, fg_real velm_axis, const fg_real* dt, hipStream_t st);
int fg_launch_balance(const fg_state* s, const FgBounds& bnd, int free_mask, fg_real atol, const fg_real* dt, hipStream_t st,
                      int outflow_mask = 0, const fg_real* outflow_velm = nullptr,
                      const fg_real* dt_host_values = nullptr);
bool fg_outflow_folds(const fg_state* s, int outflow_mask);
int fg_launch_mean_sub(const fg_state* s, const fg_real* active_dt, fg_real* p, fg_real* p_copy, hipStream_t st);

int fg_poisson_apply_launch(const fg_state* s, const fg_real* rA, const fg_real* x, fg_real* y, hipStream_t st);
int fg_poisson_jacobi_launch(const fg_state* s, const fg_real* rA, const fg_real* b, const fg_real* x, fg_real* xnew,
                             fg_real omega, hipStream_t st);
int fg_poisson_rbgs_launch(const fg_state* s, const fg_real* rA, const fg_real* b, fg_real* x, fg_real omega, int color,
                           hipStream_t st);
struct FgCgOutcome {
    const fg_real* lazy_z = nullptr;
    bool mean_ready = false;
    bool marks_valid = false;
    bool spec_done = false;
};
struct FgCgSpec { int (*fn)(void* ctx, const FgCgOutcome& o) = nullptr; void* ctx = nullptr; };
struct FgCgArgs {
    const fg_real* rA; const fg_real* b; fg_real* x;
    fg_real* r; fg_real* p; fg_real* Ap;
    const fg_real* dt;
    fg_real tol; int max_iterations; int use_x0; int reset_steps;
    int check_every;
    int precond;
    int kind = 2;
    int lazy_ok = 0;
    FgCgSpec spec;
};
int fg_cg_solve(fg_state* s, const FgCgArgs& a, fg_solve_info* info_host, hipStream_t st, FgCgOutcome* out = nullptr);

struct FgSpecHook { int (*fn)(void* ctx) = nullptr; void* ctx = nullptr; };
struct FgBicgArgs {
    const fg_real* diag; const fg_real* off;
    const fg_real* rhs; fg_real* x;
    int nc;
    const fg_real* dt;
    fg_real tol; int max_iterations; int use_x0;
    int precond = 0;
    FgNu nu; int wall_lo = 1, wall_hi = 1;
// ... 69 lines not shown
```

fluidgym_amd/csrc/fg_piso.hip:

```cpp
#include "fg_internal.h"
#include "fg_cg.h"
#include "fg_fftcg.h"

namespace {

template <int VEC>
__device__ __forceinline__ fg_real fg_elem_mask(int e, fg_real lo_mask_or_hi, bool is_edge_elem) {
    return is_edge_elem ? lo_mask_or_hi : 1.f;
}

template <int DIMS, int VEC>
__device__ __forceinline__ int fg_slab_index(const FgGrid& g, const FgCtx<DIMS, VEC>& c, int a) {
    if (a == 0) return c.k * g.ny + c.j;
    if (a == 1) return c.k * g.nx + c.i0;
    return c.j * g.nx + c.i0;
}
__device__ __forceinline__ int fg_slab_size(const FgGrid& g, int a) {
    return (a == 0) ? g.ny * g.nz : (a == 1) ? g.nx * g.nz : g.nx * g.ny;
}

template <int DIMS, int VEC, bool SCALAR, bool VISC = false>
__global__ __launch_bounds__(FG_BLOCK) void k_adv_build(FgGrid g, FgBounds bnd, FgAdvArgs a, int tiles_x,
                                                         int tiles_y, int tiles) {
    const FgCtx<DIMS, VEC> c = fg_make_ctx<DIMS, VEC>(g, tiles_x, tiles_y, tiles);
// ... 152 lines not shown
#pragma unroll
                    for (int e = 0; e < VEC; ++e) S.v[e] = a.buoy_factor * S.v[e];
                } else {
#pragma unroll
                    for (int e = 0; e < VEC; ++e) S.v[e] = 0.f;
                }
                fg_store<VEC>(a.source_w + ((size_t)c.b * DIMS + q) * N + c.idx, S);
            } else if (a.source) S = fg_load<VEC>(a.source + ((size_t)c.b * DIMS + q) * N + c.idx);
            const fg_real F = a.force ? a.force[c.b * DIMS + q] : 0.f;
#pragma unroll
            for (int e = 0; e < VEC; ++e)
                out.v[e] = (J[e] * u[q].v[e] * rdt + bsum[q][e]) * rJ[e] + ((have_s ? S.v[e] : 0.f) + F);
            fg_store<VEC>(a.rhs + ((size_t)c.b * DIMS + q) * N + c.idx, out);
        }
    }
}

__global__ __launch_bounds__(FG_BLOCK) void k_reciprocal(const fg_real* __restrict__ A, fg_real* __restrict__ rA,
                                                          const fg_real* __restrict__ dt, int n, int n4) {
    const int b = blockIdx.y;
    if (dt && !(dt[b] > 0.f)) return;
    const fg_real4* src = reinterpret_cast<const fg_real4*>(A + (size_t)b * n);
    fg_real4* dst = reinterpret_cast<fg_real4*>(rA + (size_t)b * n);
    for (int i = blockIdx.x * blockDim.x + threadIdx.x; i < n4; i += gridDim.x * blockDim.x) {
        const fg_real4 v = src[i];
        dst[i] = make_fg_real4(1.f / v.x, 1.f / v.y, 1.f / v.z, 1.f / v.w);
    }
    if (blockIdx.x == 0) {
        for (int i = n4 * 4 + threadIdx.x; i < n; i += blockDim.x) rA[(size_t)b * n + i] = 1.f / A[(size_t)b * n + i];
    }
}

template <int DIMS, int VEC>
__global__ __launch_bounds__(FG_BLOCK) void k_h(FgGrid g, const fg_real* __restrict__ dt,
                                                 const fg_real* __restrict__ rA_, const fg_real* __restrict__ Coff,
                                                 const fg_real* __restrict__ rhs, const fg_real* __restrict__ velr,
                                                 fg_real* __restrict__ hvec, FgCgBegin begin, int tiles_x, int tiles_y, int tiles) {
    const FgCtx<DIMS, VEC> c = fg_make_ctx<DIMS, VEC>(g, tiles_x, tiles_y, tiles);
    if (begin.acc && fg_xcd_remap(blockIdx.x, gridDim.x) % (unsigned)tiles == 0) fg_cg_begin_env(begin, dt, c.b);
    if (!(dt[c.b] > 0.f) || !c.valid) return;
    const size_t N = g.n;
    const FgVec<VEC> rA = fg_load<VEC>(rA_ + (size_t)c.b * N + c.idx);
    FgVec<VEC> off[2 * DIMS];
#pragma unroll
    for (int f = 0; f < 2 * DIMS; ++f) off[f] = fg_load<VEC>(Coff + ((size_t)c.b * 2 * DIMS + f) * N + c.idx);
#pragma unroll
    for (int q = 0; q < DIMS; ++q) {
        const size_t base = ((size_t)c.b * DIMS + q) * N;
        const FgNbr<DIMS, VEC> u = fg_gather<DIMS, VEC>(velr + base, c);
        const FgVec<VEC> r = fg_load<VEC>(rhs + base + c.idx);
        FgVec<VEC> out;
#pragma unroll
        for (int e = 0; e < VEC; ++e) {
            fg_real H = off[0].v[e] * u.xm.v[e] + off[1].v[e] * u.xp.v[e] + off[2].v[e] * u.ym.v[e] +
                      off[3].v[e] * u.yp.v[e];
            if constexpr (DIMS == 3) H += off[4].v[e] * u.zm.v[e] + off[5].v[e] * u.zp.v[e];
            out.v[e] = rA.v[e] * (r.v[e] - H);
        }
        fg_store<VEC>(hvec + base + c.idx, out);
    }
}

template <int DIMS, int VEC>
__global__ __launch_bounds__(FG_BLOCK) void k_div(FgGrid g, FgBounds bnd, const fg_real* __restrict__ dt,
                                                   const fg_real* __restrict__ hvec, fg_real* __restrict__ div, FgCgStart start,
                                                   int tiles_x, int tiles_y, int tiles) {
    const FgCtx<DIMS, VEC> c = fg_make_ctx<DIMS, VEC>(g, tiles_x, tiles_y, tiles);
    if (dt && !(dt[c.b] > 0.f)) return;
    if (!c.valid && !start.acc) return;
    const size_t N = g.n;
    const FgMetric<DIMS, VEC> m = fg_metrics<DIMS, VEC>(g, c);
    fg_real acc[VEC];
#pragma unroll
    for (int e = 0; e < VEC; ++e) acc[e] = 0.f;
#pragma unroll
    for (int ax = 0; ax < DIMS; ++ax) {
        FgVec<VEC> ctr, lo, hi;
        fg_gather_axis<DIMS, VEC>(hvec + ((size_t)c.b * DIMS + ax) * N, c, ax, ctr, lo, hi);
        const int slab = fg_slab_index<DIMS, VEC>(g, c, ax);
        const int slab_n = fg_slab_size(g, ax);
#pragma unroll
        for (int e = 0; e < VEC; ++e) {
            fg_real area, mask_lo, mask_hi;
            if (ax == 0) { area = m.hy * m.hz; mask_lo = (e == 0) ? c.mxm : 1.f; mask_hi = (e == VEC - 1) ? c.mxp : 1.f; }
            else if (ax == 1) { area = m.hx[e] * m.hz; mask_lo = c.mym; mask_hi = c.myp; }
            else { area = m.hx[e] * m.hy; mask_lo = c.mzm; mask_hi = c.mzp; }
            const int bi = slab + ((ax == 0) ? 0 : e);
            fg_real F_hi, F_lo;
            if (mask_hi != 0.f) F_hi = 0.5f * (ctr.v[e] + hi.v[e]) * area;
            else F_hi = bnd.vel[2 * ax + 1][((size_t)c.b * DIMS + ax) * slab_n + bi] * area;
            if (mask_lo != 0.f) F_lo = 0.5f * (ctr.v[e] + lo.v[e]) * area;
            else F_lo = bnd.vel[2 * ax][((size_t)c.b * DIMS + ax) * slab_n + bi] * area;
            acc[e] += F_hi - F_lo;
        }
    }
    FgVec<VEC> out;
#pragma unroll
    for (int e = 0; e < VEC; ++e) out.v[e] = acc[e];
    if (c.valid) fg_store<VEC>(div + (size_t)c.b * N + c.idx, out);
    if (start.acc) {
        __shared__ fg_real lds[4];
        fg_real part[1] = {0.f};
        if (c.valid) {
            FgVec<VEC> z;
#pragma unroll
            for (int e = 0; e < VEC; ++e) { z.v[e] = 0.f; part[0] += out.v[e] * out.v[e]; }
            fg_store<VEC>(start.x + (size_t)c.b * N + c.idx, z);
            fg_store<VEC>(start.r + (size_t)c.b * N + c.idx, out);
        }
        fg_block_sum<1>(part, lds);
// ... 566 lines not shown
            d += (i != j) ? 2.f * sij : sij;
        }
    out[(size_t)b * g.n + c] = coefficient * delta * FG_SQRT(2.f * d);
}

__global__ __launch_bounds__(1024) void k_wall_forcing(FgGrid g, const fg_real* __restrict__ vel, int axis, fg_real coef_lo, fg_real coef_hi,
                                                        fg_real* __restrict__ force, int dims) {
    const int b = blockIdx.x;
    const size_t N = g.n;
    const fg_real* __restrict__ u = vel + ((size_t)b * dims + axis) * N;
    double lo = 0.0, hi = 0.0;
    const int rows = g.nz;
    for (int idx = threadIdx.x; idx < rows * g.nx; idx += blockDim.x) {
        const int k = idx / g.nx, i = idx - k * g.nx;
        lo += (double)u[((size_t)k * g.ny + 0) * g.nx + i];
        hi += (double)u[((size_t)k * g.ny + (g.ny - 1)) * g.nx + i];
    }
    __shared__ double lds[2][16];
#pragma unroll
    for (int o = 32; o > 0; o >>= 1) { lo += __shfl_down(lo, o, 64); hi += __shfl_down(hi, o, 64); }
    if ((threadIdx.x & 63) == 0) { lds[0][threadIdx.x >> 6] = lo; lds[1][threadIdx.x >> 6] = hi; }
    __syncthreads();
    if (threadIdx.x == 0) {
        double sl = 0.0, sh = 0.0;
        for (int w = 0; w < (int)(blockDim.x >> 6); ++w) { sl += lds[0][w]; sh += lds[1][w]; }
        const double n = (double)rows * g.nx;
        const fg_real tau_lo = coef_lo * (fg_real)(sl / n), tau_hi = coef_hi * (fg_real)(sh / n);
        for (int q = 0; q < dims; ++q) force[b * dims + q] = (q == axis) ? (fg_real)0.5 * (tau_lo + tau_hi) : (fg_real)0;
    }
}

int fg_launch_wall_forcing(const fg_state* s, hipStream_t st) {
    hipLaunchKernelGGL(k_wall_forcing, dim3(s->grid.B), dim3(1024), 0, st, s->grid, (const fg_real*)s->velocity, s->wall_forcing_axis,
                       s->wall_forcing_coef[0], s->wall_forcing_coef[1], s->force_uniform, s->grid.dims);
    FG_HIP_CHECK(hipGetLastError());
    return FG_OK;
}

int fg_launch_sgs(const fg_state* s, const FgBounds& bnd, fg_real coefficient, fg_real* out, hipStream_t st) {
    const dim3 grid((s->grid.n + FG_BLOCK - 1) / FG_BLOCK, s->grid.B);
    if (s->grid.dims == 2) hipLaunchKernelGGL(k_sgs_smagorinsky<2>, grid, dim3(FG_BLOCK), 0, st, s->grid, bnd, (const fg_real*)s->velocity, coefficient, out);
    else hipLaunchKernelGGL(k_sgs_smagorinsky<3>, grid, dim3(FG_BLOCK), 0, st, s->grid, bnd, (const fg_real*)s->velocity, coefficient, out);
    FG_HIP_CHECK(hipGetLastError());
    return FG_OK;
}

int fg_launch_pressure_setup(const fg_state* s, const fg_real* dt, hipStream_t st) {
    const int n = s->grid.n;
    hipLaunchKernelGGL(k_reciprocal, stride_grid(s, n), dim3(FG_BLOCK), 0, st, s->A, s->rA, dt, n, (n % 4 == 0) ? n / 4 : 0);
    FG_HIP_CHECK(hipGetLastError());
    return FG_OK;
}

int fg_launch_h(fg_state* s, const fg_real* dt, const fg_real* vel_result, hipStream_t st) {
    fg_htrace("h_launch_in");
    FgCgBegin begin;
    begin.acc = s->cg_acc; begin.flags = s->flags; begin.info = s->info_dev; begin.mean_sums = s->acc; begin.best = s->cg_best;
    begin.track_best = s->cg_return_best; begin.ns = fg_cg_slots(s); begin.xsum = s->fcg_xsum;
    s->prepared.set_cg(begin.ns, begin.track_best, dt);
    const int slot_h = fg_prof_slot(s, FG_PK_H, nullptr, s->grid.B, (s->grid.dims == 3 ? 68.0 : 52.0) * (double)s->grid.n, 6.0 * s->grid.dims * s->grid.dims * (double)s->grid.n, st);
    FG_DISPATCH(s, {
        const FgLaunch L = fg_launch_geometry<DIMS, VEC>(s->grid);
        FG_LAUNCH_P(s, slot_h, (k_h<DIMS, VEC>), L.grid, dim3(FG_BLOCK), 0, st, s->grid, dt, s->rA, s->Coff, s->adv_rhs,
                    vel_result, s->hvec, begin, L.tiles_x, L.tiles_y, L.tiles);
    });
    FG_HIP_CHECK(hipGetLastError());
    fg_htrace("h_launch_out");
    return FG_OK;
}

int fg_launch_div(fg_state* s, const FgBounds& bnd, const fg_real* dt, const fg_real* hvec, fg_real* div,
                  hipStream_t st, bool cg_from_zero, bool fused_fwd) {
    FgCgStart start = {nullptr, nullptr, nullptr, 1};
    s->prepared.set_cg_start(0);
    if (cg_from_zero && dt != nullptr && s->prepared.cg_for(dt) && div == s->div) {
#if !FG_F64
        if (fused_fwd && fg_fcg_ok(s)) {
            s->prepared.set_cg_start(2);
            return fg_fcg_div_fwd(s, bnd, dt, hvec, div, s->prepared.cg_ns, st);
        }
#endif
        start.acc = s->cg_acc; start.r = s->w[0]; start.x = s->p_result; start.ns = s->prepared.cg_ns;
        s->prepared.set_cg_start(1);
    }
    const int slot_d = fg_prof_slot(s, FG_PK_DIV, nullptr, s->grid.B, 28.0 * (double)s->grid.n, 4.0 * s->grid.dims * (double)s->grid.n, st);
    FG_DISPATCH(s, {
        const FgLaunch L = fg_launch_geometry<DIMS, VEC>(s->grid);
        FG_LAUNCH_P(s, slot_d, (k_div<DIMS, VEC>), L.grid, dim3(FG_BLOCK), 0, st, s->grid, bnd, dt, hvec, div, start, L.tiles_x,
                    L.tiles_y, L.tiles);
    });
    FG_HIP_CHECK(hipGetLastError());
    return FG_OK;
}

int fg_launch_correct(const fg_state* s, const fg_real* dt, const fg_real* rA, const fg_real* hvec, const fg_real* p,
                      fg_real* vel_out, hipStream_t st, fg_real* vel_copy, const FgMeanRef* mean, const FgLazyRef* lazy) {
    fg_htrace("correct_in");
    const FgMeanRef mr = mean ? *mean : FgMeanRef{nullptr, nullptr, nullptr, nullptr, nullptr};
    const FgLazyRef lz = lazy ? *lazy : FgLazyRef{nullptr, nullptr, nullptr};
    const double cb = (s->grid.dims == 3 ? 36.0 : 28.0) + (vel_copy ? 4.0 * s->grid.dims : 0.0) + ((mean && mean->sums) || (lazy && lazy->p_res) ? 4.0 : 0.0);
    const int slot_c = fg_prof_slot(s, FG_PK_CORRECT, nullptr, s->grid.B, cb * (double)s->grid.n, 5.0 * s->grid.dims * (double)s->grid.n, st);
    FG_DISPATCH(s, {
        const FgLaunch L = fg_launch_geometry<DIMS, VEC>(s->grid);
        FG_LAUNCH_P(s, slot_c, (k_correct<DIMS, VEC>), L.grid, dim3(FG_BLOCK), 0, st, s->grid, dt, rA, hvec, p, vel_out, vel_copy, mr, lz,
                    L.tiles_x, L.tiles_y, L.tiles);
    });
    FG_HIP_CHECK(hipGetLastError());
    fg_htrace("correct_out");
    return FG_OK;
}

int fg_launch_max_velocity(const fg_state* s, const FgBounds& bnd, fg_real* out_B, hipStream_t st, fg_real* mirror_B, FgPollOut poll,
                           fg_real* flux_B, fg_real* flux_mirror, FgDtRule rule) {
    FG_REQUIRE(!rule.t_rem || (poll.gran && mirror_B && !FG_F64), FG_ERR_INVALID_ARG, "the device-side sub-step rule needs the result-word form");
    FG_REQUIRE(!flux_B || (mirror_B && flux_mirror), FG_ERR_INVALID_ARG, "the flux balance rides in the mirrored form only");
    int32_t* done_B = reinterpret_cast<int32_t*>(out_B + s->grid.B);
    FG_REQUIRE(!mirror_B || out_B == s->scratch_B + s->grid.B, FG_ERR_INVALID_ARG, "mirror needs the scratch row as out_B");
    if (!mirror_B || !s->maxvel_clean)
        FG_HIP_CHECK(hipMemsetAsync(out_B, 0, mirror_B ? sizeof(fg_real) * s->grid.B + sizeof(int32_t) * (s->grid.B + 1) : sizeof(fg_real) * s->grid.B, st));
    s->maxvel_clean = mirror_B ? 1 : 0;
    if ((s->grid.nx & 3) == 0) {
        const int rows = s->grid.ny * s->grid.nz;
        int rpb = 4;
        while ((long)((rows + 2 * rpb - 1) / (2 * rpb)) * s->grid.B >= 2048) rpb *= 2;
        while ((rows + rpb - 1) / rpb > (int)fg_reduce_wgs(s)) rpb *= 2;
        dim3 grid((rows + rpb - 1) / rpb, s->grid.B);
        const int slot_m = fg_prof_slot(s, FG_PK_MAXVEL, nullptr, s->grid.B, 4.0 * s->grid.dims * (double)s->grid.n, 2.0 * s->grid.dims * (double)s->grid.n, st);
        if (s->grid.dims == 2)
            FG_LAUNCH_P(s, slot_m, k_max_velocity_rows<2>, grid, dim3(FG_BLOCK), 0, st, s->grid, bnd, s->velocity, out_B, done_B,
                        mirror_B, rpb, poll, flux_B, flux_mirror, rule);
        else
            FG_LAUNCH_P(s, slot_m, k_max_velocity_rows<3>, grid, dim3(FG_BLOCK), 0, st, s->grid, bnd, s->velocity, out_B, done_B,
                        mirror_B, rpb, poll, flux_B, flux_mirror, rule);
        FG_HIP_CHECK(hipGetLastError());
        return FG_OK;
    }
    dim3 grid = stride_grid(s, (long)s->grid.n * 4);
    if (s->grid.dims == 2)
        hipLaunchKernelGGL(k_max_velocity<2>, grid, dim3(FG_BLOCK), 0, st, s->grid, bnd, s->velocity, out_B, done_B, mirror_B, poll, flux_B, flux_mirror, rule);
    else
        hipLaunchKernelGGL(k_max_velocity<3>, grid, dim3(FG_BLOCK), 0, st, s->grid, bnd, s->velocity, out_B, done_B, mirror_B, poll, flux_B, flux_mirror, rule);
    FG_HIP_CHECK(hipGetLastError());
    return FG_OK;
}

// ... 82 lines not shown
```

fluidgym_amd/csrc/fg_poisson.hip:

```cpp
#include <math.h>
#include <cmath>
#include <vector>

#include "fg_internal.h"
#include "fg_cg.h"
#include "fg_rung64.h"
#include "fg_fftcg.h"

namespace {

template <int DIMS, int VEC>
struct FgCoef {
    fg_real xm[VEC], xp[VEC], ym[VEC], yp[VEC], zm[VEC], zp[VEC];
};

template <int DIMS, int VEC>
__device__ __forceinline__ FgCoef<DIMS, VEC> fg_poisson_coef(const FgCtx<DIMS, VEC>& c, const FgMetric<DIMS, VEC>& m,
                                                             const FgNbr<DIMS, VEC>& rA) {
    FgCoef<DIMS, VEC> k;
    const fg_real ayz = m.hy * m.hz;
#pragma unroll
    for (int e = 0; e < VEC; ++e) {
        const fg_real rh_lo = (e == 0) ? m.rhx_m : m.rhx[e > 0 ? e - 1 : 0];
        const fg_real rh_hi = (e == VEC - 1) ? m.rhx_p : m.rhx[e < VEC - 1 ? e + 1 : VEC - 1];
// ... 205 lines not shown
    if (c.valid) {
        const FgVec<VEC> p = fg_load<VEC>(p_ + base + c.idx);
        const FgVec<VEC> Ap = fg_load<VEC>(Ap_ + base + c.idx);
        FgVec<VEC> x = fg_load<VEC>(x_ + base + c.idx);
        FgVec<VEC> r = fg_load<VEC>(r_ + base + c.idx);
        if (save) fg_store<VEC>(best.best_x + base + c.idx, x);
#pragma unroll
        for (int e = 0; e < VEC; ++e) {
            x.v[e] += alpha * p.v[e];
            r.v[e] -= alpha * Ap.v[e];
            part[0] += r.v[e] * r.v[e];
            part[1] += x.v[e];
        }
        fg_store<VEC>(x_ + base + c.idx, x);
        fg_store<VEC>(r_ + base + c.idx, r);
    }
    if (xsum) {
        const fg_real tot = fg_block_sum_lanes<2>(part, lds);
        if (threadIdx.x == 0) fg_acc_add(fg_acc_ptr(acc, c.b, (it + 1) % 3), ns, tile, (double)tot);
        if (threadIdx.x == 1) acc_add(xsum + (2 * c.b + (it & 1)), (double)tot);
    } else {
        fg_block_sum<1>(*reinterpret_cast<fg_real (*)[1]>(part), lds);
        if (threadIdx.x == 0) fg_acc_add(fg_acc_ptr(acc, c.b, (it + 1) % 3), ns, tile, (double)part[0]);
    }
}

constexpr int CG_CHECK_WAVES = 16;
__global__ __launch_bounds__(64 * CG_CHECK_WAVES) void k_cg_check(FgDacc* __restrict__ acc, int32_t* __restrict__ flags, fg_solve_info* __restrict__ info,
                                                                  fg_solve_info* __restrict__ mirror, fg_real tol, int it, int n, int B, int final_pass, int ns,
                                                                  FgPollOut poll = FgPollOut{nullptr, 0}) {
    __shared__ uint32_t stage[CG_CHECK_WAVES * 2];
    const int lane = threadIdx.x & 63, wave = threadIdx.x >> 6;
    const int b0 = blockIdx.x * CG_CHECK_WAVES, b = b0 + wave;
    const bool valid = b < B;
    if (valid && flag_ld(flags + (b)) == 0) {
        const fg_real crit = fg_rms(fg_acc_total(fg_acc_ptr(acc, b, (it + 1) % 3), ns), n);
        if (lane == 0) {
            info[b].final_residual = crit;
            info[b].used_iterations = it;
            if (!(crit >= tol)) {
                const bool finite = isfinite(crit);
                flag_st(flags + (b), finite ? 1 : 2);
                info[b].converged = finite ? 1 : 0;
                info[b].is_finite = finite ? 1 : 0;
            } else if (final_pass) {
                info[b].converged = 0;
                info[b].is_finite = 1;
            }
        }
    }
    fg_poll_publish_infos_waves(poll, mirror, info, b, valid, b0, min(CG_CHECK_WAVES, B - b0), stage);
}

__global__ void k_cg_begin(const fg_real* __restrict__ dt, FgCgBegin q, int B) {
    if ((int)blockIdx.x < B) fg_cg_begin_env(q, dt, blockIdx.x);
}

__global__ void k_zero_name(FgDacc* __restrict__ acc, int name, int B) {
    const int b = blockIdx.x;
    if (b < B && threadIdx.x < FG_CG_SLOTS) acc_st(fg_acc_ptr(acc, b, name) + threadIdx.x, 0.0);
}

__global__ __launch_bounds__(FG_BLOCK) void k_cg_restore_best(fg_real* __restrict__ x, fg_solve_info* __restrict__ info,
                                                               fg_solve_info* __restrict__ mirror, FgBest best, int n) {
    const int b = blockIdx.y;
    const fg_solve_info I = info[b];
    const fg_real have = best.saved_crit[b];
    const bool worse = !(I.final_residual <= have);
    if (I.converged || !worse || !isfinite(have)) return;
    for (int i = blockIdx.x * blockDim.x + threadIdx.x; i < n; i += gridDim.x * blockDim.x)
        x[(size_t)b * n + i] = best.best_x[(size_t)b * n + i];
    if (blockIdx.x == 0 && threadIdx.x == 0) {
        mirror[b].final_residual = have;
        mirror[b].is_finite = 1;
    }
}

}


int fg_poisson_apply_launch(const fg_state* s, const fg_real* rA, const fg_real* x, fg_real* y, hipStream_t st) {
    int zc;
    if (fg_zmarch_ok(s, &zc)) return fg_zmarch_apply(s, rA, x, y, zc, st);
    FG_DISPATCH(s, {
        const FgLaunch L = fg_launch_geometry<DIMS, VEC>(s->grid);
        hipLaunchKernelGGL((k_poisson_apply<DIMS, VEC>), L.grid, dim3(FG_BLOCK), 0, st, s->grid, rA, x, y, L.tiles_x,
                           L.tiles_y, L.tiles);
    });
    FG_HIP_CHECK(hipGetLastError());
    return FG_OK;
}

int fg_poisson_jacobi_launch(const fg_state* s, const fg_real* rA, const fg_real* b, const fg_real* x, fg_real* xnew,
                             fg_real omega, hipStream_t st) {
    int zc;
    if (fg_zmarch_ok(s, &zc)) return fg_zmarch_relax(s, rA, b, x, xnew, omega, -1, zc, st);
    FG_DISPATCH(s, {
        const FgLaunch L = fg_launch_geometry<DIMS, VEC>(s->grid);
        hipLaunchKernelGGL((k_poisson_relax<DIMS, VEC, false>), L.grid, dim3(FG_BLOCK), 0, st, s->grid, rA, b, x, xnew,
                           omega, 0, L.tiles_x, L.tiles_y, L.tiles);
    });
    FG_HIP_CHECK(hipGetLastError());
    return FG_OK;
}

int fg_poisson_rbgs_launch(const fg_state* s, const fg_real* rA, const fg_real* b, fg_real* x, fg_real omega, int color,
                           hipStream_t st) {
    int zc;
    if (fg_zmarch_ok(s, &zc)) return fg_zmarch_relax(s, rA, b, x, x, omega, color, zc, st);
    FG_DISPATCH(s, {
        const FgLaunch L = fg_launch_geometry<DIMS, VEC>(s->grid);
        hipLaunchKernelGGL((k_poisson_relax<DIMS, VEC, true>), L.grid, dim3(FG_BLOCK), 0, st, s->grid, rA, b, x, x,
                           omega, color, L.tiles_x, L.tiles_y, L.tiles);
    });
    FG_HIP_CHECK(hipGetLastError());
    return FG_OK;
}

int fg_fd_rowmean_prefactor(fg_state* s, const fg_real* dt, hipStream_t st) {
#if !FG_F64
    if (!(s->fd_Qx && fg_fcg_ok(s) && fg_fd_rowmean_ok(s)) || s->fd_row_epoch == s->rA_epoch || dt == nullptr) return FG_OK;
    const bool parts = s->fd_row_part && s->fd_row_part_epoch == s->rA_epoch;
    if (parts && fg_fd_tridiag_can_factor(s)) return FG_OK;
    if (int rc = fg_fd_rowmean_factor(s, s->rA, dt, st, parts ? s->fd_row_part : nullptr, (s->grid.nx + 63) / 64)) return rc;
    s->fd_row_epoch = s->rA_epoch;
#else
    (void)s; (void)dt; (void)st;
#endif
    return FG_OK;
}

int fg_cg_slots(const fg_state* s) {
    int tiles_per_env = 1;
    FG_DISPATCH(s, { tiles_per_env = fg_launch_geometry<DIMS, VEC>(s->grid).tiles; });
    int ns = 1;
    while (ns < FG_CG_SLOTS && tiles_per_env / ns > 256) ns *= 2;
    return ns;
}

namespace {
struct CgRun {
    int ns, nb, check_every, next_poll;
    fg_real* zvec;
    FgDacc* mean_sums;
    FgCgJudge judge;
    bool fused;
    bool start_ready = false;
    bool start_fwd = false;
    bool done = false, info_fresh = false;
};
}

static int cg_begin(fg_state* s, const FgCgArgs& a, CgRun& c, hipStream_t st) {
    const int B = s->grid.B, n = s->grid.n;
    const int ns = c.ns = fg_cg_slots(s);
    {
        const int prep = s->prepared.take_cg(ns, s->cg_return_best, a.dt);
        c.start_ready = prep > 0 && !a.use_x0 && a.b == s->div && a.r == s->w[0] && a.x == s->p_result;
        c.start_fwd = c.start_ready && prep == 2;
        if (prep < 0) {
            FgCgBegin q;
            q.acc = s->cg_acc; q.flags = s->flags; q.info = s->info_dev; q.mean_sums = s->acc; q.best = s->cg_best;
            q.track_best = s->cg_return_best; q.ns = ns; q.xsum = s->fcg_xsum;
            hipLaunchKernelGGL(k_cg_begin, dim3(B), dim3(64), 0, st, a.dt, q, B);
        }
    }
    if (!c.start_ready)
    FG_DISPATCH(s, {
        const FgLaunch L = fg_launch_geometry<DIMS, VEC>(s->grid);
        hipLaunchKernelGGL((k_cg_residual<DIMS, VEC>), L.grid, dim3(FG_BLOCK), 0, st, s->grid, a.rA, a.b, a.x, a.r,
                           s->cg_acc, s->flags, a.use_x0, 0, ns, L.tiles_x, L.tiles_y, L.tiles);
    });
    c.check_every = a.check_every > 0 ? a.check_every : 16;
    c.nb = a.precond ? 5 : 0;
    c.zvec = a.precond ? s->w[5] : a.r;
    c.judge.acc = s->cg_acc; c.judge.flags = s->flags; c.judge.info = s->info_dev; c.judge.tol = a.tol; c.judge.it = -1; c.judge.n = n; c.judge.ns = ns;
#if !FG_F64
    c.fused = a.precond && s->fd_Qx && fg_fcg_ok(s);
#else
    c.fused = false;
#endif
    if (a.precond && !c.fused) {
        if (!s->fd_Qx) { fg_set_error("preconditioned CG requested but fg_set_fd_preconditioner was not called"); return FG_ERR_INVALID_ARG; }
        if (int rc = fg_fd_apply(s, a.r, c.zvec, s->cg_acc + (size_t)(c.nb + 0) * FG_CG_SLOTS, FG_CG_NAMES * FG_CG_SLOTS, ns, B, st, &c.judge)) return rc;
    }
    c.next_poll = a.precond ? (s->pred_cg[a.kind & 3] + 1 > 1 ? s->pred_cg[a.kind & 3] + 1 : 1) : c.check_every;
    c.mean_sums = (!a.use_x0 && a.x == s->p_result && s->fcg_xsum) ? s->fcg_xsum : nullptr;
    return FG_OK;
}

#if !FG_F64
static int cg_iterate_fused(fg_state* s, const FgCgArgs& a, CgRun& c, FgCgOutcome& o, hipStream_t st) {
    const int B = s->grid.B, n = s->grid.n, ns = c.ns;
    FgCgJudge& judge = c.judge;
    FcgVectors v;
    v.x = a.x; v.r = a.r; v.t1 = s->w[3]; v.z = c.zvec; v.w = s->w[4]; v.p = a.p; v.s = a.Ap;
    FgCgLead lead;
    lead.best = s->cg_best;
    const bool rowm = fg_fd_rowmean_ok(s);
    const float* factor_from = nullptr;
    if (rowm && !(a.rA == s->rA && s->fd_row_epoch == s->rA_epoch)) {
        const bool parts = a.rA == s->rA && s->fd_row_part && s->fd_row_part_epoch == s->rA_epoch;
        if (parts && fg_fd_tridiag_can_factor(s)) factor_from = s->fd_row_part;
        else if (int rc = fg_fd_rowmean_factor(s, a.rA, a.dt, st, parts ? s->fd_row_part : nullptr, (s->grid.nx + 63) / 64)) return rc;
        s->fd_row_epoch = (a.rA == s->rA) ? s->rA_epoch : -1;
    }
    judge.it = -1;
    if (!c.start_fwd)
        if (int rc = fg_fd_dct_forward(s, a.r, v.t1, st, 0, &judge)) return rc;
    lead.judge = judge;
    if (int rc = fg_fd_tridiag(s, v.t1, st, &lead, rowm, factor_from, a.dt)) return rc;
    const fg_real* r0 = c.start_fwd ? a.b : nullptr;
    {
        FcgVectors v0 = v;
        if (r0) v0.r = const_cast<fg_real*>(r0);
        if (int rc = fg_fcg_inv_apply(s, v0, a.rA, 0, ns, st, s->fcg_first)) return rc;
    }
    if (s->fcg_first && a.max_iterations >= 1) {
        const bool poll0 = c.next_poll <= 1;
        if (poll0) fg_prof_prefetch(s, st);
        const FgPollOut po = poll0 ? fg_poll_next(&s->poll) : FgPollOut{nullptr, 0};
        if (int rc = fg_fcg_check0(s, a.tol, ns, st, po, &o.marks_valid)) return rc;
        bool spec = false;
        if (poll0 && s->fcg_spec && a.spec.fn && a.lazy_ok && r0 && c.mean_sums) {
            FgCgOutcome ahead;
            ahead.lazy_z = v.z; ahead.mean_ready = true; ahead.marks_valid = true;
            if (int rc = a.spec.fn(a.spec.ctx, ahead)) return rc;
            spec = true;
        }
        if (poll0) {
            fg_htrace("cg_check_launched");
            const int active = fg_poll_wait_active(&s->poll, po, 0, B, s->info_pinned, st);
            if (active < 0) return active;
            fg_htrace("cg_poll_done");
            c.info_fresh = true;
            s->fcg_first_polls += 1;
            if (active == 0) {
                bool all_ok = true;
                for (int b = 0; b < B; ++b) all_ok = all_ok && s->info_pinned[b].converged && s->info_pinned[b].is_finite;
                if (a.lazy_ok && r0 && all_ok && c.mean_sums) {
                    o.lazy_z = v.z; s->fcg_unstored += 1; o.spec_done = spec;
                } else {
                    if (int rc = fg_fcg_update_fwd(s, v, 0, 1, ns, st, o.marks_valid, r0)) return rc;
                }
                c.done = true;
            } else {
                c.next_poll = 2;
            }
        }
    }
    int first = 1;
    const int fused_reset = (a.reset_steps > 0 && a.reset_steps < 10) ? a.reset_steps : 10;
    for (int it = 0; it < a.max_iterations && !c.done; ++it) {
        if (int rc = fg_fcg_update_fwd(s, v, it, first, ns, st, o.marks_valid, it == 0 ? r0 : nullptr)) return rc;
        if (first) {
            fg_real* t = v.p; v.p = v.z; v.z = t;
            t = v.s; v.s = v.w; v.w = t;
            first = 0;
        }
        const bool poll = (it + 1 >= c.next_poll || it + 1 == a.max_iterations);
// ... 290 lines not shown
```

fluidgym_amd/native.py:

```python
from __future__ import annotations

import ctypes
import os
from typing import Dict, List, Optional, Sequence

import numpy as np
import torch

from . import _lib as L


def _ptr(t: Optional[torch.Tensor]):
    return None if t is None else ctypes.c_void_p(t.data_ptr())


def _stream(device) -> ctypes.c_void_p:
    return ctypes.c_void_p(torch.cuda.current_stream(device).cuda_stream)


class LinsolveError(RuntimeError):
    """A linear solve failed (reference: ``PISOtorch_diff.LinsolveError``, PISOtorch_diff.py:262)."""


class NativeSolver:

    def __init__(self, widths: Sequence[np.ndarray], batch: int, fixed_faces: Sequence[int] = (),
                 n_scalars: int = 0, scalar_bc: Optional[Dict[int, Sequence[int]]] = None,
                 device: Optional[torch.device] = None, allocate: bool = True, dtype: torch.dtype = torch.float32):
        if not torch.cuda.is_available():
            raise L.NativeLibraryError("fluidgym_amd needs a ROCm GPU (MI355X); there is no CPU path")
        if dtype not in (torch.float32, torch.float64):
            raise ValueError("dtype must be torch.float32 or torch.float64")
        self.dtype = dtype
        self.f64 = dtype == torch.float64
        self.lib = L.load_f64() if self.f64 else L.load()
        self._np_real = np.float64 if self.f64 else np.float32
        self._c_real = ctypes.c_double if self.f64 else ctypes.c_float
        self._StepOptions = L.FgStepOptionsF64 if self.f64 else L.FgStepOptions
        self._SimOptions = L.FgSimOptionsF64 if self.f64 else L.FgSimOptions
        self.device = torch.device("cuda", torch.cuda.current_device()) if device is None else torch.device(device)
        self.dims = len(widths)
        assert self.dims in (2, 3)
        self.widths = [np.ascontiguousarray(w, dtype=self._np_real) for w in widths]
        self.nx = len(self.widths[0])
        self.ny = len(self.widths[1])
        self.nz = len(self.widths[2]) if self.dims == 3 else 1
        self.n = self.nx * self.ny * self.nz
        self.B = int(batch)
        self.n_scalars = int(n_scalars)
        self.scalar_bc = {int(f): [int(t) for t in v] for f, v in (scalar_bc or {}).items()}
        self.scalar_viscosities: Dict[int, float] = {}
        self.viscosity_B: Optional[torch.Tensor] = None
        self.scalar_viscosities_B: Dict[int, Optional[torch.Tensor]] = {}
        self.fixed = [f in fixed_faces for f in range(6)]
        cfg = L.FgConfig()
        cfg.dims, cfg.nx, cfg.ny, cfg.nz = self.dims, self.nx, self.ny, self.nz
        cfg.batch, cfg.n_scalars = self.B, self.n_scalars
        cfg.device = self.device.index or 0
        for f in range(6):
            cfg.face_type[f] = L.FG_FIXED if self.fixed[f] else L.FG_PERIODIC
            for ch in range(L.FG_MAX_SCALARS):
                cfg.scalar_bc[f][ch] = L.FG_DIRICHLET
            if scalar_bc and f in scalar_bc:
                for ch, t in enumerate(scalar_bc[f]):
                    cfg.scalar_bc[f][ch] = int(t)
        fp = ctypes.POINTER(self._c_real)
        hz = self.widths[2].ctypes.data_as(fp) if self.dims == 3 else None
        handle = ctypes.c_void_p()
        L.check(self.lib.fg_create(ctypes.byref(cfg), self.widths[0].ctypes.data_as(fp),
                                   self.widths[1].ctypes.data_as(fp), hz, ctypes.byref(handle)))
        self.handle = handle
        self._bound: Dict[int, torch.Tensor] = {}
        self.viscosity = 0.0
        self.velocity = self.pressure = self.scalar = self.velocity_source = None
        self.viscosity_field = None
        self.bvel: Dict[int, torch.Tensor] = {}
        self.bscal: Dict[int, torch.Tensor] = {}
        self._dt = torch.zeros(self.B, dtype=dtype, device=self.device)
        self._dt_host = torch.zeros(self.B, dtype=dtype).pin_memory()
        self._out_B = torch.zeros(self.B, dtype=dtype, device=self.device)
        self.has_fd = bool(self.fixed[2] and self.fixed[3]) and not (self.f64 and os.environ.get("FLUIDGYM_AMD_F64_FD", "1") == "0")
        self.has_helmholtz = False
        if self.has_fd:
            fp = ctypes.POINTER(ctypes.c_float)
            from .simulation.fd_precond import FDPreconditioner

            fd = FDPreconditioner(self.widths, [f for f in range(6) if self.fixed[f]])
            fpp = lambda a: a.ctypes.data_as(fp)
            qz, qzt = (fpp(fd.Qz), fpp(fd.QzT)) if self.dims == 3 else (None, None)
            rc = self.lib.fg_set_fd_preconditioner(self.handle, fpp(fd.Qx), fpp(fd.QxT), qz, qzt, fpp(fd.lower), fpp(fd.inv), fpp(fd.cp))
            self.has_fd = rc != L.FG_ERR_UNSUPPORTED
            if self.has_fd:
                L.check(rc, lib=self.lib)
        if self.has_fd:
            no_fft = self.f64 or os.environ.get("FG_FD_NO_FFT", "0") != "0"
            if fd.x_cosine_width is not None and not no_fft:
                L.check(self.lib.fg_set_fd_fast_transform(self.handle, 0, fd.x_cosine_width), lib=self.lib)
            if fd.x_fourier_width is not None and not no_fft:
                L.check(self.lib.fg_set_fd_fast_transform(self.handle, 0, fd.x_fourier_width), lib=self.lib)
            self.has_helmholtz = bool(fd.transform_axes_periodic_uniform) and not self.f64
            if self.has_helmholtz:
                L.check(self.lib.fg_set_fd_helmholtz(self.handle, fpp(fd.lam)), lib=self.lib)
        self.default_method = L.FG_SOLVER_FDCG if self.has_fd else L.FG_SOLVER_CG
        if allocate:
            self.allocate_fields()

    @property
    def spatial(self):
        return (self.ny, self.nx) if self.dims == 2 else (self.nz, self.ny, self.nx)

    def slab(self, face: int):
        s = list(self.spatial)
        s[len(s) - 1 - (face >> 1)] = 1
        return tuple(s)

    def bind(self, field: int, t: Optional[torch.Tensor]):
        if t is not None:
            assert t.is_cuda and t.dtype == self.dtype and t.is_contiguous(), f"fields must be contiguous {self.dtype} CUDA tensors"
            self._bound[field] = t
        else:
            self._bound.pop(field, None)
        L.check(self.lib.fg_bind(self.handle, field, _ptr(t)), lib=self.lib)

    def allocate_fields(self):
# ... 259 lines not shown
                                              int(bool(signed_components)), _stream(self.device)), lib=self.lib)

    def env_reset_solver_state(self, sel):
        self._env_sel = sel
        L.check(self.lib.fg_env_reset_solver_state(self.handle, sel, len(sel), _stream(self.device)), lib=self.lib)

    def make_divergence_free(self, tol=1e-5, max_iterations=1000):
        info = self._infos(self.B)
        rc = self.lib.fg_make_divergence_free(self.handle, tol, max_iterations, info, _stream(self.device))
        L.check(rc, allow=(L.FG_ERR_NOT_CONVERGED,))
        return list(info)

    def poisson_apply(self, rA, x, y=None):
        y = torch.empty_like(x) if y is None else y
        L.check(self.lib.fg_poisson_apply(self.handle, _ptr(rA), _ptr(x), _ptr(y), _stream(self.device)), lib=self.lib)
        return y

    def poisson_jacobi(self, rA, b, x, sweeps, omega=1.0):
        L.check(self.lib.fg_poisson_jacobi(self.handle, _ptr(rA), _ptr(b), _ptr(x), sweeps, omega, _stream(self.device)), lib=self.lib)
        return x

    def poisson_rbgs(self, rA, b, x, sweeps, omega=1.0):
        L.check(self.lib.fg_poisson_rbgs(self.handle, _ptr(rA), _ptr(b), _ptr(x), sweeps, omega, _stream(self.device)), lib=self.lib)
        return x

    def poisson_cg(self, rA, b, x, tol=1e-5, max_iterations=5000, use_x0=False):
        info = self._infos(self.B)
        rc = self.lib.fg_poisson_cg(self.handle, _ptr(rA), _ptr(b), _ptr(x), tol, max_iterations, int(use_x0), info,
                                    _stream(self.device))
        L.check(rc, allow=(L.FG_ERR_NOT_CONVERGED, L.FG_ERR_NOT_FINITE))
        return list(info)


    def solver_counters(self, reset: bool = False) -> dict:
        unconv = (ctypes.c_int64 * 4)()
        L.check(self.lib.fg_solver_unconverged(self.handle, unconv))
        out = (ctypes.c_int64 * 13)()
        L.check(self.lib.fg_solver_counters(self.handle, out, int(reset)), lib=self.lib)
        names = ("scalar", "velocity", "pressure0", "pressure1")
        res = {n: {"mean": (out[k] / out[4 + k]) if out[4 + k] else None, "max": int(out[8 + k]), "systems": int(out[4 + k]),
                    "unconverged": int(unconv[k])}
               for k, n in enumerate(names)}
        res["piso_steps"] = int(out[12])
        return res

    def config_dump(self) -> dict:
        out = L.read_json(self.lib.fg_config_dump, self.handle, lib=self.lib)
        out["env"] = {k: v for k, v in sorted(os.environ.items()) if k.startswith(("FG_", "FLUIDGYM_"))}
        return out

    def set_return_best(self, on: bool = True):
        L.check(self.lib.fg_set_return_best(self.handle, int(on)), lib=self.lib)

    def set_cg_reset_steps(self, steps: int = 100):
        L.check(self.lib.fg_set_cg_reset_steps(self.handle, int(steps)), lib=self.lib)

    def set_advection_start(self, from_result: bool = True):
        L.check(self.lib.fg_set_advection_start(self.handle, int(from_result)), lib=self.lib)

    def set_wall_stress_forcing(self, axis: int, coef_lo: float = 0.0, coef_hi: float = 0.0) -> None:
        L.check(self.lib.fg_set_wall_stress_forcing(self.handle, int(axis), float(coef_lo), float(coef_hi)), lib=self.lib)

    def set_advection_preconditioner(self, mode: int = 0):
        L.check(self.lib.fg_set_advection_preconditioner(self.handle, int(mode)), lib=self.lib)

    def apply_advection_preconditioner(self, mode: int, r: torch.Tensor, return_forms: bool = False):
        r = r.to(self.device, self.dtype).contiguous()
        z = torch.empty_like(r)
        forms = (ctypes.c_int32 * L.FG_FORM_SLOTS)()
        L.check(self.lib.fg_debug_apply_preconditioner(self.handle, int(mode), int(r.shape[1]), ctypes.c_void_p(r.data_ptr()),
                                                       ctypes.c_void_p(z.data_ptr()), forms, _stream(self.device)), lib=self.lib)
        return (z, list(forms)) if return_forms else z

    def apply_pressure_preconditioner(self, form: int, r: torch.Tensor, rA: Optional[torch.Tensor] = None):
        r = r.to(self.device, self.dtype).contiguous()
        z = torch.empty_like(r)
        ra = ctypes.c_void_p(None) if rA is None else ctypes.c_void_p(rA.data_ptr())
        rz = (ctypes.c_double * self.B)()
        forms = (ctypes.c_int32 * L.FG_FORM_SLOTS)()
        L.check(self.lib.fg_debug_apply_pressure_preconditioner(self.handle, int(form), ra, ctypes.c_void_p(r.data_ptr()),
                                                                ctypes.c_void_p(z.data_ptr()), rz, forms, _stream(self.device)),
                lib=self.lib)
        return z, list(rz), list(forms)

    def advection_retries(self, reset: bool = False) -> int:
        out = ctypes.c_int64()
        L.check(self.lib.fg_advection_retries(self.handle, ctypes.byref(out), int(reset)), lib=self.lib)
        return int(out.value)

    def set_double_fallback(self, on: bool = True) -> None:
        L.check(self.lib.fg_set_double_fallback(self.handle, int(bool(on))), lib=self.lib)

    def set_advection_jacobi(self, on: bool = True) -> None:
        L.check(self.lib.fg_set_advection_jacobi(self.handle, int(bool(on))), lib=self.lib)

    def advection_jacobi_counts(self) -> Dict[str, int]:
        out = (ctypes.c_int64 * 2)()
        L.check(self.lib.fg_advection_jacobi_counts(self.handle, out), lib=self.lib)
        return {"settled_by_sweeps": int(out[0]), "handed_to_bicgstab": int(out[1])}

    def ladder(self, force_mask: int = -1) -> Dict[str, int]:
        out = (ctypes.c_int64 * 4)()
        L.check(self.lib.fg_ladder(self.handle, out, int(force_mask)), lib=self.lib)
        return {"advection_fp64": int(out[0]), "advection_preconditioned": int(out[1]), "pressure_fp64": int(out[2])}

    def advection_solver_form(self, nc: Optional[int] = None) -> str:
# ... 53 lines not shown
```

include/fluidgym_hip.h:

```cpp
#ifndef FLUIDGYM_HIP_H
#define FLUIDGYM_HIP_H

#include <stdint.h>

#ifdef __cplusplus
extern "C" {
#endif

#define FG_ABI_VERSION 1

#ifdef FG_REAL_DOUBLE
typedef double fg_real;
#else
typedef float fg_real;
#endif
#define FG_MAX_SCALARS 4

#define FG_OK 0
#define FG_ERR_INVALID_ARG (-1)
#define FG_ERR_NOT_BOUND (-2)
#define FG_ERR_HIP (-3)
#define FG_ERR_UNSUPPORTED (-4)
#define FG_ERR_NOT_CONVERGED (-5)
#define FG_ERR_NOT_FINITE (-6)
// ... 7 lines not shown
enum fg_field {
    FG_VELOCITY = 0,
    FG_PRESSURE = 1,
    FG_SCALAR = 2,
    FG_VELOCITY_SOURCE = 3,
    FG_VISCOSITY_FIELD = 4,
    FG_BOUND_VELOCITY = 8,
    FG_BOUND_SCALAR = 16
};

#define FG_SOLVER_CG 0
#define FG_SOLVER_JACOBI 1
#define FG_SOLVER_RBGS 2
#define FG_SOLVER_MGCG 3
#define FG_SOLVER_FDCG 4

typedef struct fg_state* fg_handle;

typedef struct fg_config {
    int32_t dims;
    int32_t nx, ny, nz;
    int32_t batch;
    int32_t n_scalars;
    int32_t face_type[6];
    int32_t scalar_bc[6][FG_MAX_SCALARS];
    int32_t device;
} fg_config;

typedef struct fg_solve_info {
    float final_residual;
    int32_t used_iterations;
    int32_t converged;
    int32_t is_finite;
} fg_solve_info;

int fg_abi_version(void);
const char* fg_last_error(void);

int fg_create(const fg_config* cfg, const fg_real* hx_host, const fg_real* hy_host, const fg_real* hz_host,
              fg_handle* out);
int fg_destroy(fg_handle h);

int fg_bind(fg_handle h, int field, fg_real* ptr);
int fg_set_viscosity(fg_handle h, fg_real viscosity);
int fg_set_scalar_viscosity(fg_handle h, int channel, fg_real viscosity);
int fg_set_viscosity_batch(fg_handle h, const fg_real* nu_B);
int fg_set_scalar_viscosity_batch(fg_handle h, int channel, const fg_real* k_B);

int fg_set_fd_preconditioner(fg_handle h, const float* Qx_host, const float* QxT_host, const float* Qz_host,
                             const float* QzT_host, const float* lower_host, const float* inv_host,
                             const float* cp_host);
int fg_set_fd_fast_transform(fg_handle h, int axis, float cell_width);
int fg_set_return_best(fg_handle h, int on);
int fg_set_cg_reset_steps(fg_handle h, int steps);
int fg_set_advection_start(fg_handle h, int from_result);
int fg_set_wall_stress_forcing(fg_handle h, int axis, fg_real coef_lo, fg_real coef_hi);

int fg_max_velocity(fg_handle h, fg_real* out_B, void* stream);
int fg_boundary_flux_balance(fg_handle h, fg_real* out_B, void* stream);

int fg_step_diagnostics(fg_handle h, fg_real* out_host_2B, void* stream);
int fg_update_advective_boundary(fg_handle h, int face, const fg_real* velm_host, const fg_real* dt_B, void* stream);
int fg_balance_boundary_fluxes(fg_handle h, int free_face_mask, fg_real atol, const fg_real* dt_B, void* stream);

int fg_setup_advection(fg_handle h, const fg_real* dt_B, int for_scalar, int channel, void* stream);
int fg_solve_advection(fg_handle h, int for_scalar, int channel, fg_real tol, int max_iterations,
                       fg_solve_info* info_host, void* stream);
int fg_set_advection_preconditioner(fg_handle h, int mode);
int fg_sgs_smagorinsky(fg_handle h, fg_real coefficient, fg_real* out_BN, void* stream);
#define FG_DIAG_GRADIENT 0
#define FG_DIAG_VORTICITY 1
#define FG_DIAG_VORTICITY_MAGNITUDE 2
#define FG_DIAG_Q 3
#define FG_DIAG_STRAIN_NORM 4
int fg_flow_diagnostic(fg_handle h, int kind, fg_real* out, void* stream);
int fg_debug_apply_preconditioner(fg_handle h, int mode, int nc, const fg_real* r, fg_real* z, int32_t* forms_out, void* stream);
int fg_debug_apply_pressure_preconditioner(fg_handle h, int form, const fg_real* rA, const fg_real* r, fg_real* z, double* rz_out,
                                           int32_t* forms_out, void* stream);
#define FG_FORM_SLOTS 8
#define FG_FORM_SLOT_X 0
#define FG_FORM_SLOT_Z 1
#define FG_FORM_SLOT_TRIDIAG 2
#define FG_FORM_SLOT_FACTORS 3
#define FG_FORM_SLOT_HELM 4
#define FG_FORM_SLOT_LINE 5
#define FG_FORM_GEMM_SPLITK 1
#define FG_FORM_GEMM_T64 2
#define FG_FORM_GEMM_T128 3
#define FG_FORM_GEMM_Z64 4
#define FG_FORM_DCT 5
#define FG_FORM_FFT 6
#define FG_FORM_F64 7
#define FG_FORM_TRI_STREAM 1
#define FG_FORM_TRI_LDS3 2
#define FG_FORM_TRI_LDS2 3
#define FG_FORM_TRI_LDS3_FAC 4
#define FG_FORM_TRI_LDS2_FAC 5
#define FG_FORM_TRI_F64 6
#define FG_FORM_FAC_GRID 1
#define FG_FORM_FAC_ROWMEAN 2
#define FG_FORM_FAC_MADE 3
#define FG_FORM_HELM_ARRAY 1
#define FG_FORM_HELM_ROW32 2
#define FG_FORM_HELM_ROW64 3
#define FG_FORM_LINE_LDS 1
#define FG_FORM_LINE_STREAM 2
// ... 390 lines not shown
```

profiles/gen_switch_table.py:

```python
import os
import re
import sys

ROOT = os.path.dirname(os.path.dirname(os.path.abspath(__file__)))

TABLE = os.path.join("fluidgym_amd", "csrc", "fg_switches.h")
ENTRY = re.compile(r'X\((FG_\w+), ([\w.]+), (-?\d+), (\w+), (HANDLE|PROCESS), (no|bits|policy), "(.*)"\)')

NOTES = {
    "FLUIDGYM_AMD_ADVECTION_JACOBI": ("policy", "policy advection_jacobi (default 1): the Simulation asks for the Jacobi sweeps of fg_jacobi.hip on the grids that qualify"),
    "FLUIDGYM_AMD_PRESSURE_REFINEMENT": ("bits", "policy pressure_refinement (default 0 = off): up to N mixed-precision corrections behind every single-block pressure solve (fp64 residual, fp32 corrections: fg_set_pressure_refinement) -- an accuracy mode"),
    "FLUIDGYM_AMD_MULTI_STEP": ("no", "0: the sim steps of an env step are issued one by one from Python instead of through fg_multi_step (A/B runs; same bits)"),
    "FLUIDGYM_AMD_F64_FD": ("bits", "0: the fp64 library solves the pressure systems with the reference's plain CG instead of the CG preconditioned by the fast-diagonalisation operator in doubles (csrc/fg_f64_fd.hip; A/B runs: iterations per solve)"),
    "FLUIDGYM_AMD_ENV_GLUE": ("bits", "0: ChannelJet2D's action schedule and reward / observation as elementwise torch launches instead of the two native kernels of fg_envglue.hip (A/B runs; the schedule is bit-identical, the means differ by fp32 rounding of the summation order)"),
    "FLUIDGYM_AMD_LANES": ("no", "default of ParallelFluidEnv(lanes=...): sub-batches of a rank's env batch, each its own solver handle, stepped concurrently by that many host threads on their own HIP streams (1 = one batch; bench.py passes --lanes 2).  Same bits per env as the sub-batches stepped alone"),
    "FG_FD_NO_FFT": ("bits", "1: the x basis change of the FD preconditioner as dense GEMM instead of the row FFT (tests)"),
    "FLUIDGYM_AMD_LIB": ("no", "path of libfluidgym_hip.so (sanitizer build: tests/run_sanitizer_suite.sh)"),
    "FLUIDGYM_AMD_LIB_F64": ("no", "path of libfluidgym_hip_f64.so"),
    "FLUIDGYM_AMD_ADVECTION_FD_PRECONDITIONER": ("bits", "policy advection_fd_preconditioner: auto (2-D periodic-x grids) / always / never"),
    "FLUIDGYM_AMD_ADVECTION_LINE_PRECONDITIONER": ("bits", "policy advection_line_preconditioner (off)"),
    "FLUIDGYM_AMD_ADVECTION_RUNG_PRECONDITIONER": ("bits", "preconditioner of the BiCG_precondition_fallback rung: line / ilu"),
    "FLUIDGYM_AMD_ADVECTION_WARM_START": ("policy", "1: velocity solve starts from the current velocity in both branches (reference: branch rule)"),
    "FLUIDGYM_AMD_PRESSURE_WARM_START": ("policy", "1: pressure solves start from the previous pressure (reference: zero)"),
    "FLUIDGYM_AMD_PRESSURE_STALL_ACCEPT": ("policy", "accept a stalled pressure solve within a factor of the tolerance (off)"),
    "FLUIDGYM_AMD_PRESSURE_MULTILEVEL": ("bits", "multilevel preconditioner of the multi-block pressure CG"),
    "FLUIDGYM_AMD_PRESSURE_MULTILEVEL_BICGSTAB": ("bits", "multilevel trial of the airfoil's refined BiCGStab"),
    "FLUIDGYM_AMD_PRESSURE_MULTILEVEL_FP64": ("bits", "policy pressure_multilevel_fp64 (default 0): float64 cylinder / airfoil envs on 2-D meshes install the multilevel preconditioner in the fp64 build (kernel-form preconditioned CG, unfused BiCGStab trial) instead of the plain recurrences"),
    "FLUIDGYM_AMD_PRESSURE_BICGSTAB_LARGE_MESHES": ("bits", "3-D multi-block ids take the refined BiCGStab"),
    "FLUIDGYM_AMD_NATIVE_WALL_FORCING": ("bits", "policy native_wall_forcing: the TCF forcing hook runs inside the library"),
    "FLUIDGYM_COLLECTIVE_TIMEOUT_S": ("no", "timeout of ParallelFluidEnv's process group (600 s)"),
    "FLUIDGYM_FORCE_COLLECTIVES": ("no", "ParallelFluidEnv issues its collectives at world size 1 too (tests)"),
    "FLUIDGYM_MASTER_PORT": ("no", "rendezvous port of the reference-style ParallelFluidEnv(cuda_ids=...) entry"),
    "FLUIDGYM_DATA_PATH": ("no", "local data path (initial domains), as config.update('local_data_path', ...)"),
}
IGNORE = {"RANK", "WORLD_SIZE", "LOCAL_RANK", "MASTER_ADDR", "MASTER_PORT", "HSA_ENABLE_IPC_MODE_LEGACY", "PYTHONPATH", "OMP_NUM_THREADS",
          "OPENBLAS_NUM_THREADS", "MKL_NUM_THREADS", "TMPDIR", "GRAFT_REPO_ROOT"}


def native_rows():
    rows = {}
    for no, line in enumerate(open(os.path.join(ROOT, TABLE)), 1):
        for m in ENTRY.finditer(line):
            rows[m.group(1)] = (m.group(6), m.group(7), m.group(5), f"{TABLE}:{no}")
    return rows


def scan():
    found = {name: [row[3]] for name, row in native_rows().items()}
    for base, _, files in os.walk(os.path.join(ROOT, "fluidgym_amd")):
        if "_san" in base or "_f64" in base or "_var" in base or "__pycache__" in base:
            continue
        for fn in files:
            if not fn.endswith((".hip", ".h", ".py")):
                continue
            path = os.path.join(base, fn)
            rel = os.path.relpath(path, ROOT)
            for no, line in enumerate(open(path, errors="replace"), 1):
                for m in re.finditer(r'getenv\("([A-Z][A-Z0-9_]+)"\)', line):
                    found.setdefault(m.group(1), []).append(f"{rel}:{no}")
                for m in re.finditer(r'environ(?:\.get)?[\[(]\s*"([A-Z][A-Z0-9_]+)"', line):
                    found.setdefault(m.group(1), []).append(f"{rel}:{no}")
    return {k: v for k, v in found.items() if k not in IGNORE}


def render(found):
    lines = ["# Environment switches of fluidgym_amd", "",
# ... 43 lines not shown
```

Before: 10470 env-steps/s.

## Fuse H operator, divergence and first FD transform into one kernel

Measured after the change: 10430 env-steps/s (median of 2 runs). About the same (-0.4%).

```diff
diff --git a/fluidgym_amd/_lib.py b/fluidgym_amd/_lib.py
--- a/fluidgym_amd/_lib.py
+++ b/fluidgym_amd/_lib.py
@@ -286,6 +286,7 @@
     "fg_max_velocity": (c_int, [c_void_p, c_void_p, c_void_p]),
     "fg_set_fd_fast_transform": (c_int, [c_void_p, c_int, c_float]),
     "fg_set_return_best": (c_int, [c_void_p, c_int]),
+    "fg_set_fused_pressure_rhs": (c_int, [c_void_p, c_int]),
     "fg_set_cg_reset_steps": (c_int, [c_void_p, c_int]),
     "fg_set_advection_start": (c_int, [c_void_p, c_int]),
     "fg_set_wall_stress_forcing": (c_int, [c_void_p, c_int, c_float, c_float]),
diff --git a/fluidgym_amd/csrc/fg_api.hip b/fluidgym_amd/csrc/fg_api.hip
--- a/fluidgym_amd/csrc/fg_api.hip
+++ b/fluidgym_amd/csrc/fg_api.hip
@@ -129,10 +129,13 @@
     FG_HIP_CHECK(hipMalloc(&s->fcg_lazy, sizeof(int32_t) * (size_t)g.B));
     FG_HIP_CHECK(hipMemset(s->fcg_lazy, 0, sizeof(int32_t) * (size_t)g.B));
     s->cg_return_best = 1;
+    s->fused_rhs = 1;
     s->cg_reset_steps = 100;
     s->adv_from_result = 1;
     FG_HIP_CHECK(hipMalloc(&s->cg_acc, sizeof(FgDacc) * (size_t)g.B * 8 * 64));
     FG_HIP_CHECK(hipMemset(s->cg_acc, 0, sizeof(FgDacc) * (size_t)g.B * 8 * 64));
+    FG_HIP_CHECK(hipMalloc(&s->rr_start, sizeof(FgDacc) * 2 * (size_t)g.B * 64));
+    FG_HIP_CHECK(hipMemset(s->rr_start, 0, sizeof(FgDacc) * 2 * (size_t)g.B * 64));
     FG_HIP_CHECK(hipMalloc(&s->cg_best.best_crit, sizeof(fg_real) * g.B));
     FG_HIP_CHECK(hipMalloc(&s->cg_best.saved_crit, sizeof(fg_real) * g.B));
     FG_HIP_CHECK(hipMalloc(&s->cg_best.save_at, sizeof(int32_t) * g.B));
@@ -156,7 +159,7 @@
     float* fd[] = {s->fd_Qx, s->fd_QxT, s->fd_Qz, s->fd_QzT, s->fd_lower, s->fd_inv, s->fd_cp};
     for (float* p : fd) if (p) (void)hipFree(p);
     if (s->fd_dct_tw) { (void)hipFree(s->fd_dct_tw); (void)hipFree(s->fd_dct_rot); }
-    (void)hipFree(s->cg_acc); (void)hipFree(s->fcg_alpha); (void)hipFree(s->fcg_xsum); (void)hipFree(s->fcg_lazy);
+    (void)hipFree(s->cg_acc); (void)hipFree(s->rr_start); (void)hipFree(s->fcg_alpha); (void)hipFree(s->fcg_xsum); (void)hipFree(s->fcg_lazy);
     if (s->jac_prev) (void)hipHostFree(s->jac_prev);
     (void)hipFree(s->fd_row_part); (void)hipFree(s->fd_lam_x); (void)hipFree(s->fd_row_inv); (void)hipFree(s->fd_row_cp); (void)hipFree(s->fd_row_lower);
     (void)hipFree(s->line_inv); (void)hipFree(s->line_cp); (void)hipFree(s->ilu_d);
@@ -239,6 +242,12 @@
 extern "C" int fg_set_return_best(fg_handle s, int on) {
     FG_REQUIRE(s, FG_ERR_INVALID_ARG, "null handle");
     s->cg_return_best = on ? 1 : 0;
+    return FG_OK;
+}
+
+extern "C" int fg_set_fused_pressure_rhs(fg_handle s, int on) {
+    FG_REQUIRE(s, FG_ERR_INVALID_ARG, "null handle");
+    s->fused_rhs = on ? 1 : 0;
     return FG_OK;
 }
 
@@ -536,9 +545,8 @@
 static int spec_h(void* p) {
     const SpecH* c = static_cast<const SpecH*>(p);
     fg_state* s = c->s;
-    if (int rc = fg_launch_h(s, c->dt, s->vel_result, c->st)) return rc;
-    return fg_launch_div(s, make_bounds(s, 0), c->dt, s->hvec, s->div, c->st, !c->opt->pressure_warm_start,
-                         c->opt->pressure_method == FG_SOLVER_FDCG && s->fd_Qx != nullptr);
+    return fg_launch_hdiv(s, make_bounds(s, 0), c->dt, s->vel_result, c->st, !c->opt->pressure_warm_start,
+                          c->opt->pressure_method == FG_SOLVER_FDCG && s->fd_Qx != nullptr);
 }
 
 static int launch_corrector(fg_state* s, const fg_real* dt, const FgCgOutcome& o, bool last, hipStream_t st) {
@@ -734,9 +742,8 @@
         FgRange range_corr(c == 0 ? "pressure_corrector_0" : "pressure_corrector_1+");
         const bool last = (c + 1 == opt->corrector_steps);
         if (!(c == 0 && h_div_ran)) {
-            if (int rc = fg_launch_h(s, dt_B, s->vel_result, st)) return rc;
-            if (int rc = fg_launch_div(s, make_bounds(s, 0), dt_B, s->hvec, s->div, st, !opt->pressure_warm_start,
-                                       opt->pressure_method == FG_SOLVER_FDCG && s->fd_Qx != nullptr))
+            if (int rc = fg_launch_hdiv(s, make_bounds(s, 0), dt_B, s->vel_result, st, !opt->pressure_warm_start,
+                                        opt->pressure_method == FG_SOLVER_FDCG && s->fd_Qx != nullptr))
                 return rc;
         }
         SpecCorrect spec_ctx = {s, dt_B, last, st};
@@ -763,7 +770,8 @@
         {"fast_transform_x", s->fd_dct_x}, {"fd_preconditioner", s->fd_Qx ? 1 : 0}, {"helmholtz", s->fd_lam ? 1 : 0}, {"advection_preconditioner", s->adv_precond},
         {"advection_from_result", s->adv_from_result}, {"return_best", s->cg_return_best}, {"cg_reset_steps", s->cg_reset_steps}, {"double_fallback", s->double_fallback},
         {"wall_forcing_axis", s->wall_forcing_axis}, {"first_iterate_polls", s->fcg_first_polls}, {"unstored_pressure_solves", s->fcg_unstored},
-        {"jacobi_speculation_misses", s->jac_spec_missed}, {"jacobi_floor_released", s->jac_floor_released}, {"pressure_refinement_corrections", s->ref64_corrections}};
+        {"jacobi_speculation_misses", s->jac_spec_missed}, {"jacobi_floor_released", s->jac_floor_released}, {"pressure_refinement_corrections", s->ref64_corrections},
+        {"fused_pressure_rhs", s->fused_rhs}, {"fused_pressure_rhs_launches", (long long)s->hdiv_launches}};
     for (const auto& kv : state) fg_json_put(out, kv.first, kv.second);
     return fg_json_out(out + "}", buf, n);
 }
@@ -941,6 +949,7 @@
     FG_REQUIRE(s && s->velocity, FG_ERR_NOT_BOUND, "velocity not bound");
     for (int k = 0; k < 4; ++k) s->jac_hist[k] = FgJacHist{0, 0, 0};
     FG_HIP_CHECK(hipMemsetAsync(s->p_result, 0, sizeof(fg_real) * (size_t)s->grid.B * s->grid.n, (hipStream_t)stream));
+    FG_HIP_CHECK(hipMemsetAsync(s->rr_start, 0, sizeof(FgDacc) * 2 * (size_t)s->grid.B * 64, (hipStream_t)stream));
     return fg_launch_copy_active(s, nullptr, s->velocity, s->vel_result, s->grid.dims, (hipStream_t)stream);
 }
 
diff --git a/fluidgym_amd/csrc/fg_cg.h b/fluidgym_amd/csrc/fg_cg.h
--- a/fluidgym_amd/csrc/fg_cg.h
+++ b/fluidgym_amd/csrc/fg_cg.h
@@ -53,10 +53,14 @@
     FgDacc* acc;
     int32_t* flags; fg_solve_info* info;
     fg_real tol; int it, n, ns;
+    const FgDacc* start = nullptr;
 };
 #ifdef __HIPCC__
+__device__ __forceinline__ const FgDacc* fg_cg_judge_rr(const FgCgJudge& j, int b) {
+    return (j.start && j.it == -1) ? j.start + (size_t)b * FG_CG_SLOTS : fg_acc_ptr(j.acc, b, (j.it + 1) % 3);
+}
 __device__ __forceinline__ bool fg_cg_judge(const FgCgJudge& j, int b, bool leader) {
-    const double rr = fg_acc_total(fg_acc_ptr(j.acc, b, (j.it + 1) % 3), j.ns);
+    const double rr = fg_acc_total(fg_cg_judge_rr(j, b), j.ns);
     const fg_real crit = (fg_real)sqrt(rr / (double)j.n);
     if (crit >= j.tol) return false;
     if (leader) {
@@ -75,7 +79,7 @@
 #ifdef __HIPCC__
 __device__ __forceinline__ bool fg_cg_lead(const FgCgLead& q, int b, bool lead_block) {
     const FgCgJudge& j = q.judge;
-    const double rr = fg_acc_total(fg_acc_ptr(j.acc, b, (j.it + 1) % 3), j.ns);
+    const double rr = fg_acc_total(fg_cg_judge_rr(j, b), j.ns);
     const fg_real crit = (fg_real)sqrt(rr / (double)j.n);
     const bool done = !(crit >= j.tol);
     if (lead_block && threadIdx.x < 64) {
diff --git a/fluidgym_amd/csrc/fg_fftcg.h b/fluidgym_amd/csrc/fg_fftcg.h
--- a/fluidgym_amd/csrc/fg_fftcg.h
+++ b/fluidgym_amd/csrc/fg_fftcg.h
@@ -34,7 +34,16 @@
     const float* hx; const float* hy; int fixed_x;
 };
 
+struct FcgHdivArgs {
+    FcgDivArgs d;
+    const float* rA; const float* Coff; const float* rhs; const float* u;
+    float* hvec;
+    FgCgBegin begin;
+    FgDacc* rr; FgDacc* rr_next;
+};
+
 #if !FG_F64
+int fg_fcg_hdiv_fwd(fg_state* s, const FgBounds& bnd, const fg_real* dt, const fg_real* vel_result, const FgCgBegin& begin, hipStream_t st);
 int fg_fcg_div_fwd(fg_state* s, const FgBounds& bnd, const fg_real* dt, const fg_real* hvec, fg_real* div, int ns, hipStream_t st);
 bool fg_fcg_ok(const fg_state* s);
 int fg_fcg_update_fwd(fg_state* s, const FcgVectors& v, int it, int first, int ns, hipStream_t st, bool marks_valid, const fg_real* r0 = nullptr);
diff --git a/fluidgym_amd/csrc/fg_fftcg.hip b/fluidgym_amd/csrc/fg_fftcg.hip
--- a/fluidgym_amd/csrc/fg_fftcg.hip
+++ b/fluidgym_amd/csrc/fg_fftcg.hip
@@ -383,6 +383,154 @@
     if (threadIdx.x == 0) fg_acc_add(fg_acc_ptr(a.acc, b, 0), a.ns, blockIdx.x, (double)part[0]);
 }
 
+template <int N>
+__device__ __forceinline__ void fcg_div_row(const FcgDivArgs& a, int b, int j, int lane, const float* hxr, const float* hyc,
+                                            const float* hyu, const float* hyd, float (&out)[N / 64]) {
+    using M = Map<N>;
+    constexpr int VW = M::VW;
+    const bool live = j < a.rows;
+    const int jc = live ? j : 0;
+    const float hy = a.hy[jc];
+    const bool at_lo = jc == 0, at_hi = jc == a.rows - 1;
+#pragma unroll
+    for (int q = 0; q < M::NG; ++q) {
+        const int i0 = q * 64 * VW + lane * VW;
+        float hc[VW], v1[VW], vu[VW], vd[VW], hx[VW], bl[VW], bh[VW];
+        fgfft::ldv<VW>(hxr + i0, hc);
+        fgfft::ldv<VW>(hyc + i0, v1);
+        fgfft::ldv<VW>(hyu + i0, vu);
+        fgfft::ldv<VW>(hyd + i0, vd);
+        fgfft::ldv<VW>(a.hx + i0, hx);
+        if (at_lo) fgfft::ldv<VW>(a.bvel[2] + ((size_t)b * 2 + 1) * N + i0, bl);
+        if (at_hi) fgfft::ldv<VW>(a.bvel[3] + ((size_t)b * 2 + 1) * N + i0, bh);
+        const float hl = hxr[(i0 == 0) ? N - 1 : i0 - 1], hr = hxr[(i0 + VW == N) ? 0 : i0 + VW];
+        const bool xlo = (i0 == 0) && a.fixed_x, xhi = (i0 + VW == N) && a.fixed_x;
+        if constexpr (VW == 4) {
+            constexpr int form[2][4] = {{0, 0, 1, 1}, {1, 1, 0, 1}};
+            float t[5];
+            t[0] = xlo ? a.bvel[0][((size_t)b * 2 + 0) * a.rows + jc] : 0.5f * (hc[0] + hl);
+            t[1] = 0.5f * (hc[0] + hc[1]); t[2] = 0.5f * (hc[1] + hc[2]); t[3] = 0.5f * (hc[2] + hc[3]);
+            t[4] = xhi ? a.bvel[1][((size_t)b * 2 + 0) * a.rows + jc] : 0.5f * (hc[3] + hr);
+#pragma unroll
+            for (int e = 0; e < 4; ++e) {
+                const float fx = form[q & 1][e] ? __builtin_fmaf(hy, t[e + 1], -(hy * t[e])) : __builtin_fmaf(-hy, t[e], hy * t[e + 1]);
+                const float u_hi = at_hi ? bh[e] : 0.5f * (v1[e] + vd[e]), u_lo = at_lo ? bl[e] : 0.5f * (v1[e] + vu[e]);
+                const float fy = __builtin_fmaf(hx[e], u_hi, -(hx[e] * u_lo));
+                const float acc = (0.f + fx) + fy;
+                out[q * VW + e] = live ? acc : 0.f;
+            }
+            continue;
+        }
+#pragma unroll
+        for (int e = 0; e < VW; ++e) {
+            const float h_l = (e == 0) ? hl : hc[e > 0 ? e - 1 : 0], h_r = (e == VW - 1) ? hr : hc[e < VW - 1 ? e + 1 : VW - 1];
+            float acc = 0.f;
+            {
+                const float area = hy;
+                const float F_hi = (e == VW - 1 && xhi) ? a.bvel[1][((size_t)b * 2 + 0) * a.rows + jc] * area : 0.5f * (hc[e] + h_r) * area;
+                const float F_lo = (e == 0 && xlo) ? a.bvel[0][((size_t)b * 2 + 0) * a.rows + jc] * area : 0.5f * (hc[e] + h_l) * area;
+                acc += F_hi - F_lo;
+            }
+            {
+                const float area = hx[e];
+                const float F_hi = at_hi ? bh[e] * area : 0.5f * (v1[e] + vd[e]) * area;
+                const float F_lo = at_lo ? bl[e] * area : 0.5f * (v1[e] + vu[e]) * area;
+                acc += F_hi - F_lo;
+            }
+            out[q * VW + e] = live ? acc : 0.f;
+        }
+    }
+}
+
+template <int N, bool PERIODIC>
+__global__ __launch_bounds__(320) void k_fcg_hdiv_fwd(FcgHdivArgs a) {
+    constexpr int EPL = N / 64;
+    using M = Map<N>;
+    constexpr int VW = M::VW;
+    __shared__ __attribute__((aligned(16))) float2 buf[2][4][N];
+    __shared__ __attribute__((aligned(16))) float2 twl[N];
+    __shared__ __attribute__((aligned(16))) float hys[10][N];
+    __shared__ float red[8];
+    const FcgDivArgs& d = a.d;
+    const int b = blockIdx.y;
+    if (blockIdx.x == 0) {
+        fg_cg_begin_env(a.begin, d.dt, b);
+        if ((int)threadIdx.x < d.ns) acc_st(a.rr_next + (size_t)b * FG_CG_SLOTS + threadIdx.x, 0.0);
+    }
+    if (!(d.dt[b] > 0.f)) return;
+    const int lane = threadIdx.x & 63, wave = threadIdx.x >> 6;
+    for (int k = threadIdx.x; k < N; k += 320) twl[k] = d.tw[k];
+    const int j0 = blockIdx.x * 8, row0 = j0 + 2 * wave;
+    float* sx = reinterpret_cast<float*>(buf[1][wave < 4 ? wave : 0]);
+#pragma unroll
+    for (int half = 0; half < 2; ++half) {
+        const int j = wave < 4 ? row0 + half : (half ? j0 + 8 : j0 - 1);
+        const int slot = wave < 4 ? 1 + 2 * wave + half : (half ? 9 : 0);
+        const bool live = j >= 0 && j < d.rows;
+        const int jc = live ? j : 0;
+        const int jm = jc == 0 ? jc : jc - 1, jp = jc == d.rows - 1 ? jc : jc + 1;
+        const size_t row = (size_t)jc * N;
+#pragma unroll
+        for (int q = 0; q < M::NG; ++q) {
+            const int i0 = q * 64 * VW + lane * VW;
+            const int il = (i0 == 0) ? (d.fixed_x ? 0 : N - 1) : i0 - 1, ir = (i0 + VW == N) ? (d.fixed_x ? N - 1 : 0) : i0 + VW;
+            float rA[VW], off[4][VW];
+            fgfft::ldv<VW>(a.rA + (size_t)b * d.n + row + i0, rA);
+#pragma unroll
+            for (int f = 0; f < 4; ++f) fgfft::ldv<VW>(a.Coff + ((size_t)b * 4 + f) * d.n + row + i0, off[f]);
+#pragma unroll
+            for (int c = 1; c >= 0; --c) {
+                if (c == 0 && wave == 4) continue;
+                const float* u = a.u + ((size_t)b * 2 + c) * d.n;
+                float uc[VW], um[VW], up[VW], r[VW], h[VW];
+                fgfft::ldv<VW>(u + row + i0, uc);
+                fgfft::ldv<VW>(u + (size_t)jm * N + i0, um);
+                fgfft::ldv<VW>(u + (size_t)jp * N + i0, up);
+                fgfft::ldv<VW>(a.rhs + ((size_t)b * 2 + c) * d.n + row + i0, r);
+                const float ul = u[row + il], ur = u[row + ir];
+#pragma unroll
+                for (int e = 0; e < VW; ++e) {
+                    const float u_l = (e == 0) ? ul : uc[e > 0 ? e - 1 : 0], u_r = (e == VW - 1) ? ur : uc[e < VW - 1 ? e + 1 : VW - 1];
+                    h[e] = fg_h_cell(rA[e], r[e], fg_h_sum_xy(off[0][e], off[1][e], off[2][e], off[3][e], u_l, u_r, um[e], up[e]));
+                    if (!live) h[e] = 0.f;
+                }
+                if (live && wave < 4) fgfft::stv<VW>(a.hvec + ((size_t)b * 2 + c) * d.n + row + i0, h);
+                fgfft::stv<VW>((c ? hys[slot] : sx + half * N) + i0, h);
+            }
+        }
+    }
+    __syncthreads();
+    float da[EPL], db[EPL];
+    float part[1] = {0.f};
+    if (wave < 4) {
+#pragma unroll
+        for (int half = 0; half < 2; ++half) {
+            const int j = row0 + half;
+            const int slot = 1 + 2 * wave + half;
+            float (&out)[EPL] = half ? db : da;
+            fcg_div_row<N>(d, b, j, lane, sx + half * N, hys[slot], hys[slot - 1], hys[slot + 1], out);
+            if (j < d.rows) {
+#pragma unroll
+                for (int e = 0; e < EPL; ++e) {
+                    float sq = out[e] * out[e];
+#if defined(__HIP_DEVICE_COMPILE__)
+                    if constexpr (VW == 4) asm volatile("" : "+v"(sq));
+#endif
+                    part[0] += sq;
+                }
+                fgfft::store_row<N>(d.div + (size_t)b * d.n + (size_t)j * N, lane, out);
+            }
+        }
+        fgfft::wave_sync();
+        float oa[EPL], ob[EPL];
+        fgfft::forward_rows<N, PERIODIC>(da, db, oa, ob, buf[0][wave], buf[1][wave], twl, d.rot, fgfft::Scales{d.fs0, d.fs}, lane);
+        if (row0 < d.rows) fgfft::store_row<N>(d.t1 + (size_t)b * d.n + (size_t)row0 * N, lane, oa);
+        if (row0 + 1 < d.rows) fgfft::store_row<N>(d.t1 + (size_t)b * d.n + (size_t)(row0 + 1) * N, lane, ob);
+    }
+    fg_block_sum<1>(part, red);
+    if (threadIdx.x == 0) fg_acc_add(a.rr + (size_t)b * FG_CG_SLOTS, d.ns, blockIdx.x, (double)part[0]);
+}
+
 template <bool PERIODIC>
 int launch_upd(const fg_state* s, int slot, int n, const FcgUpdArgs& a, dim3 grid, hipStream_t st) {
     switch (n) {
@@ -414,6 +562,19 @@
         case 128: FG_LAUNCH_P(s, slot, (k_fcg_div_fwd<128, PERIODIC>), grid, dim3(256), 0, st, a); break;
         case 256: FG_LAUNCH_P(s, slot, (k_fcg_div_fwd<256, PERIODIC>), grid, dim3(256), 0, st, a); break;
         case 512: FG_LAUNCH_P(s, slot, (k_fcg_div_fwd<512, PERIODIC>), grid, dim3(256), 0, st, a); break;
+        default: fg_set_error("fused CG: unsupported row length"); return FG_ERR_UNSUPPORTED;
+    }
+    return FG_OK;
+}
+
+template <bool PERIODIC>
+int launch_hdiv(const fg_state* s, int n, const FcgHdivArgs& a, dim3 grid, hipStream_t st) {
+    const int slot = fg_prof_slot(s, FG_PK_DIV, nullptr, s->grid.B, 52.0 * (double)s->grid.n, (24.0 + 8.0 + 5.0 * log2((double)n)) * (double)s->grid.n, st);
+    switch (n) {
+        case 64: FG_LAUNCH_P(s, slot, (k_fcg_hdiv_fwd<64, PERIODIC>), grid, dim3(320), 0, st, a); break;
+        case 128: FG_LAUNCH_P(s, slot, (k_fcg_hdiv_fwd<128, PERIODIC>), grid, dim3(320), 0, st, a); break;
+        case 256: FG_LAUNCH_P(s, slot, (k_fcg_hdiv_fwd<256, PERIODIC>), grid, dim3(320), 0, st, a); break;
+        case 512: FG_LAUNCH_P(s, slot, (k_fcg_hdiv_fwd<512, PERIODIC>), grid, dim3(320), 0, st, a); break;
         default: fg_set_error("fused CG: unsupported row length"); return FG_ERR_UNSUPPORTED;
     }
     return FG_OK;
@@ -465,7 +626,7 @@
     *marks_valid = true;
     return FG_OK;
 }
-int fg_fcg_div_fwd(fg_state* s, const FgBounds& bnd, const fg_real* dt, const fg_real* hvec, fg_real* div, int ns, hipStream_t st) {
+static FcgDivArgs fcg_div_args(const fg_state* s, const FgBounds& bnd, const fg_real* dt, const fg_real* hvec, fg_real* div, int ns) {
     const FgGrid& G = s->grid;
     FcgDivArgs a = {};
     a.h = hvec; a.div = div; a.r = s->w[0]; a.x = s->p_result; a.t1 = s->w[3];
@@ -473,6 +634,24 @@
     a.tw = s->fd_dct_tw; a.rot = s->fd_dct_rot; a.fs0 = s->fd_dct_fwd[0]; a.fs = s->fd_dct_fwd[1];
     a.dt = dt; a.acc = s->cg_acc; a.ns = ns; a.rows = G.ny; a.n = G.n;
     a.hx = G.h[0]; a.hy = G.h[1]; a.fixed_x = G.fixed[0];
+    return a;
+}
+int fg_fcg_hdiv_fwd(fg_state* s, const FgBounds& bnd, const fg_real* dt, const fg_real* vel_result, const FgCgBegin& begin, hipStream_t st) {
+    const FgGrid& G = s->grid;
+    FcgHdivArgs a = {};
+    a.d = fcg_div_args(s, bnd, dt, nullptr, s->div, begin.ns);
+    a.rA = s->rA; a.Coff = s->Coff; a.rhs = s->adv_rhs; a.u = vel_result; a.hvec = s->hvec; a.begin = begin;
+    const size_t half = (size_t)G.B * FG_CG_SLOTS;
+    a.rr = s->rr_start + (s->hdiv_launches & 1u) * half;
+    a.rr_next = s->rr_start + ((s->hdiv_launches + 1u) & 1u) * half;
+    const dim3 grid((G.ny + 7) / 8, G.B);
+    if (int rc = (s->fd_dct_x == 2 ? launch_hdiv<true>(s, G.nx, a, grid, st) : launch_hdiv<false>(s, G.nx, a, grid, st))) return rc;
+    FG_HIP_CHECK(hipGetLastError());
+    return FG_OK;
+}
+int fg_fcg_div_fwd(fg_state* s, const FgBounds& bnd, const fg_real* dt, const fg_real* hvec, fg_real* div, int ns, hipStream_t st) {
+    const FgGrid& G = s->grid;
+    const FcgDivArgs a = fcg_div_args(s, bnd, dt, hvec, div, ns);
     const dim3 grid((G.ny + 7) / 8, G.B);
     if (int rc = (s->fd_dct_x == 2 ? launch_div<true>(s, G.nx, a, grid, st) : launch_div<false>(s, G.nx, a, grid, st))) return rc;
     FG_HIP_CHECK(hipGetLastError());
diff --git a/fluidgym_amd/csrc/fg_internal.h b/fluidgym_amd/csrc/fg_internal.h
--- a/fluidgym_amd/csrc/fg_internal.h
+++ b/fluidgym_amd/csrc/fg_internal.h
@@ -326,6 +326,12 @@
     return n;
 }
 
+__device__ __forceinline__ fg_real fg_h_sum_xy(fg_real o_xm, fg_real o_xp, fg_real o_ym, fg_real o_yp, fg_real u_xm, fg_real u_xp,
+                                               fg_real u_ym, fg_real u_yp) {
+    return o_xm * u_xm + o_xp * u_xp + o_ym * u_ym + o_yp * u_yp;
+}
+__device__ __forceinline__ fg_real fg_h_cell(fg_real rA, fg_real rhs, fg_real H) { return rA * (rhs - H); }
+
 template <int DIMS, int VEC>
 __device__ __forceinline__ void fg_gather_axis(const fg_real* __restrict__ q, const FgCtx<DIMS, VEC>& c, int axis,
                                                FgVec<VEC>& ctr, FgVec<VEC>& lo, FgVec<VEC>& hi) {
@@ -582,14 +588,17 @@
     int bicg_nc; const fg_real* bicg_dt;
     int cg_ns, cg_best; const fg_real* cg_dt;
     int cg_start;
+    const FgDacc* cg_rr;
     void clear() { *this = FgPrepared{}; }
     void set_bicg(int nc, const fg_real* dt) { clear(); bicg_nc = nc; bicg_dt = dt; }
     void set_cg(int ns, int best, const fg_real* dt) { clear(); cg_ns = ns; cg_best = best; cg_dt = dt; }
     bool cg_for(const fg_real* dt) const { return cg_ns > 0 && cg_dt == dt; }
-    void set_cg_start(int form) { cg_start = form; }
+    void set_cg_start(int form, const FgDacc* rr = nullptr) { cg_start = form; cg_rr = rr; }
     bool take_bicg(int nc, const fg_real* dt) { const bool ready = bicg_nc == nc && bicg_dt == dt; clear(); return ready; }
-    int take_cg(int ns, int best, const fg_real* dt) {
-        const int got = (cg_ns == ns && cg_best == best && cg_dt == dt) ? cg_start : -1; clear(); return got;
+    int take_cg(int ns, int best, const fg_real* dt, const FgDacc** rr = nullptr) {
+        const int got = (cg_ns == ns && cg_best == best && cg_dt == dt) ? cg_start : -1;
+        if (rr) *rr = got > 0 ? cg_rr : nullptr;
+        clear(); return got;
     }
 };
 
@@ -646,6 +655,7 @@
     FG_SB_SWITCHES(FG_SW_MEMBER)
     double* fcg_alpha; FgDacc* fcg_xsum;
     int32_t* fcg_lazy;
+    int fused_rhs; FgDacc* rr_start; unsigned hdiv_launches;
     long jac_spec_missed;
     long jac_floor_released = 0;
     long fcg_unstored, fcg_first_polls;
@@ -762,6 +772,8 @@
 int fg_launch_div(fg_state* s, const FgBounds& bnd, const fg_real* dt, const fg_real* hvec, fg_real* div, hipStream_t st,
                   bool cg_from_zero = false,
                   bool fused_fwd = false);
+int fg_launch_hdiv(fg_state* s, const FgBounds& bnd, const fg_real* dt, const fg_real* vel_result, hipStream_t st, bool cg_from_zero,
+                   bool fused_fwd);
 struct FgMeanRef { const FgDacc* sums; const fg_solve_info* info; fg_real* p_copy; const int32_t* lazy; const double* alpha; };
 struct FgLazyRef { const int32_t* lazy; const double* alpha; fg_real* p_res; };
 int fg_launch_correct(const fg_state* s, const fg_real* dt, const fg_real* rA, const fg_real* hvec, const fg_real* p,
diff --git a/fluidgym_amd/csrc/fg_piso.hip b/fluidgym_amd/csrc/fg_piso.hip
--- a/fluidgym_amd/csrc/fg_piso.hip
+++ b/fluidgym_amd/csrc/fg_piso.hip
@@ -228,10 +228,9 @@
         FgVec<VEC> out;
 #pragma unroll
         for (int e = 0; e < VEC; ++e) {
-            fg_real H = off[0].v[e] * u.xm.v[e] + off[1].v[e] * u.xp.v[e] + off[2].v[e] * u.ym.v[e] +
-                      off[3].v[e] * u.yp.v[e];
+            fg_real H = fg_h_sum_xy(off[0].v[e], off[1].v[e], off[2].v[e], off[3].v[e], u.xm.v[e], u.xp.v[e], u.ym.v[e], u.yp.v[e]);
             if constexpr (DIMS == 3) H += off[4].v[e] * u.zm.v[e] + off[5].v[e] * u.zp.v[e];
-            out.v[e] = rA.v[e] * (r.v[e] - H);
+            out.v[e] = fg_h_cell(rA.v[e], r.v[e], H);
         }
         fg_store<VEC>(hvec + base + c.idx, out);
     }
@@ -904,11 +903,16 @@
     return FG_OK;
 }
 
-int fg_launch_h(fg_state* s, const fg_real* dt, const fg_real* vel_result, hipStream_t st) {
-    fg_htrace("h_launch_in");
+static FgCgBegin cg_begin_args(fg_state* s) {
     FgCgBegin begin;
     begin.acc = s->cg_acc; begin.flags = s->flags; begin.info = s->info_dev; begin.mean_sums = s->acc; begin.best = s->cg_best;
     begin.track_best = s->cg_return_best; begin.ns = fg_cg_slots(s); begin.xsum = s->fcg_xsum;
+    return begin;
+}
+
+int fg_launch_h(fg_state* s, const fg_real* dt, const fg_real* vel_result, hipStream_t st) {
+    fg_htrace("h_launch_in");
+    const FgCgBegin begin = cg_begin_args(s);
     s->prepared.set_cg(begin.ns, begin.track_best, dt);
     const int slot_h = fg_prof_slot(s, FG_PK_H, nullptr, s->grid.B, (s->grid.dims == 3 ? 68.0 : 52.0) * (double)s->grid.n, 6.0 * s->grid.dims * s->grid.dims * (double)s->grid.n, st);
     FG_DISPATCH(s, {
@@ -943,6 +947,24 @@
     });
     FG_HIP_CHECK(hipGetLastError());
     return FG_OK;
+}
+
+int fg_launch_hdiv(fg_state* s, const FgBounds& bnd, const fg_real* dt, const fg_real* vel_result, hipStream_t st, bool cg_from_zero,
+                   bool fused_fwd) {
+#if !FG_F64
+    if (s->fused_rhs && cg_from_zero && fused_fwd && dt != nullptr && fg_fcg_ok(s)) {
+        fg_htrace("h_launch_in");
+        const FgCgBegin begin = cg_begin_args(s);
+        if (int rc = fg_fcg_hdiv_fwd(s, bnd, dt, vel_result, begin, st)) return rc;
+        s->prepared.set_cg(begin.ns, begin.track_best, dt);
+        s->prepared.set_cg_start(2, s->rr_start + (size_t)(s->hdiv_launches & 1u) * s->grid.B * FG_CG_SLOTS);
+        s->hdiv_launches += 1;
+        fg_htrace("h_launch_out");
+        return FG_OK;
+    }
+#endif
+    if (int rc = fg_launch_h(s, dt, vel_result, st)) return rc;
+    return fg_launch_div(s, bnd, dt, s->hvec, s->div, st, cg_from_zero, fused_fwd);
 }
 
 int fg_launch_correct(const fg_state* s, const fg_real* dt, const fg_real* rA, const fg_real* hvec, const fg_real* p,
diff --git a/fluidgym_amd/csrc/fg_poisson.hip b/fluidgym_amd/csrc/fg_poisson.hip
--- a/fluidgym_amd/csrc/fg_poisson.hip
+++ b/fluidgym_amd/csrc/fg_poisson.hip
@@ -281,8 +281,14 @@
     fg_poll_publish_infos_waves(poll, mirror, info, b, valid, b0, min(CG_CHECK_WAVES, B - b0), stage);
 }
 
-__global__ void k_cg_begin(const fg_real* __restrict__ dt, FgCgBegin q, int B) {
-    if ((int)blockIdx.x < B) fg_cg_begin_env(q, dt, blockIdx.x);
+__global__ void k_cg_begin(const fg_real* __restrict__ dt, FgCgBegin q, int B, FgDacc* __restrict__ rr_start) {
+    const int b = blockIdx.x;
+    if (b >= B) return;
+    fg_cg_begin_env(q, dt, b);
+    if (rr_start && (int)threadIdx.x < q.ns) {
+        acc_st(rr_start + (size_t)b * FG_CG_SLOTS + threadIdx.x, 0.0);
+        acc_st(rr_start + ((size_t)B + b) * FG_CG_SLOTS + threadIdx.x, 0.0);
+    }
 }
 
 __global__ void k_zero_name(FgDacc* __restrict__ acc, int name, int B) {
@@ -376,6 +382,7 @@
     bool fused;
     bool start_ready = false;
     bool start_fwd = false;
+    const FgDacc* rr_start = nullptr;
     bool done = false, info_fresh = false;
 };
 }
@@ -384,14 +391,16 @@
     const int B = s->grid.B, n = s->grid.n;
     const int ns = c.ns = fg_cg_slots(s);
     {
-        const int prep = s->prepared.take_cg(ns, s->cg_return_best, a.dt);
+        const FgDacc* rr = nullptr;
+        const int prep = s->prepared.take_cg(ns, s->cg_return_best, a.dt, &rr);
         c.start_ready = prep > 0 && !a.use_x0 && a.b == s->div && a.r == s->w[0] && a.x == s->p_result;
         c.start_fwd = c.start_ready && prep == 2;
+        c.rr_start = c.start_fwd ? rr : nullptr;
         if (prep < 0) {
             FgCgBegin q;
             q.acc = s->cg_acc; q.flags = s->flags; q.info = s->info_dev; q.mean_sums = s->acc; q.best = s->cg_best;
             q.track_best = s->cg_return_best; q.ns = ns; q.xsum = s->fcg_xsum;
-            hipLaunchKernelGGL(k_cg_begin, dim3(B), dim3(64), 0, st, a.dt, q, B);
+            hipLaunchKernelGGL(k_cg_begin, dim3(B), dim3(64), 0, st, a.dt, q, B, s->rr_start);
         }
     }
     if (!c.start_ready)
@@ -435,6 +444,7 @@
         s->fd_row_epoch = (a.rA == s->rA) ? s->rA_epoch : -1;
     }
     judge.it = -1;
+    judge.start = c.rr_start;
     if (!c.start_fwd)
         if (int rc = fg_fd_dct_forward(s, a.r, v.t1, st, 0, &judge)) return rc;
     lead.judge = judge;
diff --git a/fluidgym_amd/native.py b/fluidgym_amd/native.py
--- a/fluidgym_amd/native.py
+++ b/fluidgym_amd/native.py
@@ -70,6 +70,8 @@
         L.check(self.lib.fg_create(ctypes.byref(cfg), self.widths[0].ctypes.data_as(fp),
                                    self.widths[1].ctypes.data_as(fp), hz, ctypes.byref(handle)))
         self.handle = handle
+        if os.environ.get("FLUIDGYM_AMD_FUSED_PRESSURE_RHS", "1") == "0":
+            L.check(self.lib.fg_set_fused_pressure_rhs(self.handle, 0), lib=self.lib)
         self._bound: Dict[int, torch.Tensor] = {}
         self.viscosity = 0.0
         self.velocity = self.pressure = self.scalar = self.velocity_source = None
@@ -435,6 +437,9 @@
     def set_return_best(self, on: bool = True):
         L.check(self.lib.fg_set_return_best(self.handle, int(on)), lib=self.lib)
 
+    def set_fused_pressure_rhs(self, on: bool = True):
+        L.check(self.lib.fg_set_fused_pressure_rhs(self.handle, int(on)), lib=self.lib)
+
     def set_cg_reset_steps(self, steps: int = 100):
         L.check(self.lib.fg_set_cg_reset_steps(self.handle, int(steps)), lib=self.lib)
 
diff --git a/include/fluidgym_hip.h b/include/fluidgym_hip.h
--- a/include/fluidgym_hip.h
+++ b/include/fluidgym_hip.h
@@ -83,6 +83,7 @@
                              const float* cp_host);
 int fg_set_fd_fast_transform(fg_handle h, int axis, float cell_width);
 int fg_set_return_best(fg_handle h, int on);
+int fg_set_fused_pressure_rhs(fg_handle h, int on);
 int fg_set_cg_reset_steps(fg_handle h, int steps);
 int fg_set_advection_start(fg_handle h, int from_result);
 int fg_set_wall_stress_forcing(fg_handle h, int axis, fg_real coef_lo, fg_real coef_hi);
diff --git a/profiles/gen_switch_table.py b/profiles/gen_switch_table.py
--- a/profiles/gen_switch_table.py
+++ b/profiles/gen_switch_table.py
@@ -12,6 +12,7 @@
     "FLUIDGYM_AMD_PRESSURE_REFINEMENT": ("bits", "policy pressure_refinement (default 0 = off): up to N mixed-precision corrections behind every single-block pressure solve (fp64 residual, fp32 corrections: fg_set_pressure_refinement) -- an accuracy mode"),
     "FLUIDGYM_AMD_MULTI_STEP": ("no", "0: the sim steps of an env step are issued one by one from Python instead of through fg_multi_step (A/B runs; same bits)"),
     "FLUIDGYM_AMD_F64_FD": ("bits", "0: the fp64 library solves the pressure systems with the reference's plain CG instead of the CG preconditioned by the fast-diagonalisation operator in doubles (csrc/fg_f64_fd.hip; A/B runs: iterations per solve)"),
+    "FLUIDGYM_AMD_FUSED_PRESSURE_RHS": ("no", "0: every solver handle is created with fg_set_fused_pressure_rhs(0) -- H operator and divergence / first transform of each pressure solve of the PISO step as two launches (k_h, k_fcg_div_fwd) instead of one (k_fcg_hdiv_fwd); A/B runs, same bits"),
     "FLUIDGYM_AMD_ENV_GLUE": ("bits", "0: ChannelJet2D's action schedule and reward / observation as elementwise torch launches instead of the two native kernels of fg_envglue.hip (A/B runs; the schedule is bit-identical, the means differ by fp32 rounding of the summation order)"),
     "FLUIDGYM_AMD_LANES": ("no", "default of ParallelFluidEnv(lanes=...): sub-batches of a rank's env batch, each its own solver handle, stepped concurrently by that many host threads on their own HIP streams (1 = one batch; bench.py passes --lanes 2).  Same bits per env as the sub-batches stepped alone"),
     "FG_FD_NO_FFT": ("bits", "1: the x basis change of the FD preconditioner as dense GEMM instead of the row FFT (tests)"),
```
